# tkeskita/smoothMesh

Hardware: AMD Instinct MI355X
Metric: mesh-points smoothed/sec/node (100 iters) + achieved HBM GB/s vs roofline (higher is better)
Workload: dtype f64

## Files before the change

### smoothmesh_amd/csrc/smgpu.hip

```cpp
#include <hip/hip_runtime.h>
#include <hip/hip_ext.h>

#include <algorithm>
#include <chrono>
#include <future>
#include <memory>
#include <mutex>
#include <cstdio>
#include <cstring>
#include <string>
#include <vector>

#include "kernels.hpp"
#include "layers.hpp"
#include "kernels_tiled.hpp"
#include "kernels_walk.hpp"
#include "kernels_filter.hpp"
#include "kernels_boundary.hpp"
#include "kernels_quality.hpp"
#include "boundary.hpp"
#include "tiles.hpp"
#include "topology.hpp"
#include "parallel.hpp"

// ... 154 lines not shown
    hipStream_t bndSide = nullptr;
    hipEvent_t evBndFork = nullptr, evBndJoin = nullptr;
    bool bndPreInFlight = false;
    bool bndPending = false, bndNormalsFromLayers = false;
    std::vector<double> bndPts, bndSurfPts;
    std::vector<int32_t> bndSurfTris;
    std::vector<uint8_t> bndFlags, bndInternal;
    std::vector<BndPatch> bndPatches;
    double bndBlend = 0.0;
    BndView bv{};
    BoundarySetup bs;
    std::vector<int32_t> layerHopsHost, layerMapHost;
    bool useExch = false;
    hipStream_t exch = nullptr;
    hipEvent_t evToExch = nullptr, evFromExch = nullptr;
    bool faFilterInFlight = false;
    EdgeTiles etl;
    EdgeTileView ev{};
    bool edgeTilesOk = false;
    size_t avgPackedCount = 0;
    size_t edgeLds = 0;
    bool eaCoop = true;
    int eaMaxEntries = 0;
    int *qOwn = nullptr, *qNei = nullptr;
    QFace* qFacePart = nullptr;
    QCell* qCellPart = nullptr;
    smgpu_quality* qOut = nullptr;
    int *qProcFace = nullptr, *qSlot = nullptr;
    int qNProc = 0, qNotCounted = 0, qCountedProc = 0;
    std::vector<int32_t> qCoupling;
    smgpu_quality_part* qPartOut = nullptr;
    uint64_t qEpoch = 1, qPackEpoch = 0;
    bool iterOpen = false;
};

static int envInt(const char* name, int def) {
    const char* v = std::getenv(name);
    return v ? std::atoi(v) : def;
}

static int sideStreamDefault(int64_t nPoints) {
    const char* v = std::getenv("ROCPROF_COUNTER_COLLECTION");
    if (v && std::atoi(v) != 0) return 0;
    return nPoints <= (int64_t)envInt("SMGPU_SIDE_STREAM_MAX_POINTS", 4000000) ? 1 : 0;
}


template <typename T>
static int devAlloc(smgpu_handle* h, T** out, size_t n) {
    void* p = nullptr;
    const size_t bytes = std::max<size_t>(n, 1) * sizeof(T);
    HIP_OK(hipMalloc(&p, bytes));
    h->allocs.push_back(p);
    h->deviceBytes += (int64_t)bytes;
    *out = (T*)p;
    return 0;
}
template <typename T>
static int devUpload(smgpu_handle* h, const T** out, const std::vector<T>& v) {
    T* p = nullptr;
    if (devAlloc(h, &p, v.size())) return 1;
    if (!v.empty()) HIP_OK(hipMemcpy(p, v.data(), v.size() * sizeof(T), hipMemcpyHostToDevice));
    *out = p;
    return 0;
}

static Prm makePrm(const smgpu_handle* h) {
    const smgpu_params& p = h->prm;
    Prm r;
    r.layersOn = h->layersOn ? 1 : 0;
    r.bndOn = h->bndOn ? 1 : 0;
    r.maxStep = p.maxStepLength;
    r.relStepFrac = p.relStepFrac;
    r.minEdge = p.minEdgeLength;
    r.totalMinFreeze = p.totalMinFreeze;
    r.smallAngle = SMGPU_PI * p.minAngle / 180.0;
    r.largeAngle = SMGPU_PI * p.maxAngle / 180.0;
    const double M = (double)kFaMargin + 2.0e-5;
    r.faCosLo = (r.smallAngle >= SMGPU_PI) ? -2.0f : (float)(std::cos(std::max(r.smallAngle, 0.0)) - M);
    r.faCosHi = (r.largeAngle <= 0.0) ? 2.0f : (float)(std::cos(std::min(r.largeAngle, SMGPU_PI)) + M);
    static const long long nearUlps = [] { const char* e = std::getenv("SMGPU_NEARTIE_ULPS"); return e ? std::max(0ll, std::atoll(e)) : 4ll; }();
    r.nearUlps = nearUlps;
    return r;
}

static inline int gridFor(int64_t n) { return (int)((n + kBlock - 1) / kBlock); }

template <typename F>
static int launchK(smgpu_handle* h, int k, F&& f, hipStream_t stream = nullptr) {
    if (!stream) stream = h->stream;
    if (h->timing) {
        hipEvent_t a, b;
        for (hipEvent_t* ev : {&a, &b}) {
            if (!h->freeEvents.empty()) { *ev = h->freeEvents.back(); h->freeEvents.pop_back(); }
            else HIP_OK(hipEventCreate(ev));
        }
        HIP_OK(hipEventRecord(a, stream));
        f();
        HIP_OK(hipEventRecord(b, stream));
        h->pending.push_back({k, a, b});
    } else {
        f();
    }
    const hipError_t le = hipGetLastError();
    if (le != hipSuccess) return fail(std::string("launch of ") + kKernelNames[k] + ": " + hipGetErrorString(le));
    h->launches[k]++;
    return 0;
}

template <typename F>
static int launchKDispatch(smgpu_handle* h, int k, F&& f) {
    if (h->timing) {
        hipEvent_t a, b;
        for (hipEvent_t* ev : {&a, &b}) {
            if (!h->freeEvents.empty()) { *ev = h->freeEvents.back(); h->freeEvents.pop_back(); }
            else HIP_OK(hipEventCreate(ev));
        }
        f(a, b);
        h->pending.push_back({k, a, b});
    } else {
        f((hipEvent_t) nullptr, (hipEvent_t) nullptr);
    }
    const hipError_t le = hipGetLastError();
    if (le != hipSuccess) return fail(std::string("launch of ") + kKernelNames[k] + ": " + hipGetErrorString(le));
    h->launches[k]++;
    return 0;
}

static hipError_t zeroNow(void* p, int v, size_t bytes) {
    hipError_t e = hipMemset(p, v, bytes);
    return e != hipSuccess ? e : hipStreamSynchronize(nullptr);
}

enum { DEP_FORK = 0, DEP_JOIN = 1, DEP_TO_EXCH = 2, DEP_FROM_EXCH = 3, DEP_BND_FORK = 4, DEP_BND_JOIN = 5, DEP_COUNT = 6 };
static int depInit(smgpu_handle* h) {
    if (h->depWords || !envInt("SMGPU_STREAM_OPS", 1)) return 0;
    int can = 0;
    if (hipDeviceGetAttribute(&can, hipDeviceAttributeCanUseStreamWaitValue, h->device) != hipSuccess || !can) { (void)hipGetLastError(); return 0; }
    if (hipMalloc((void**)&h->depWords, DEP_COUNT * 64) != hipSuccess) { (void)hipGetLastError(); h->depWords = nullptr; return 0; }
    if (zeroNow(h->depWords, 0, DEP_COUNT * 64) != hipSuccess) return fail("hipMemset failed");
    h->streamOps = true;
    return 0;
}
static int depSignal(smgpu_handle* h, int kind, hipStream_t from, hipEvent_t ev) {
    if (h->streamOps) {
        if (hipStreamWriteValue32(from, h->depWords + 16 * kind, ++h->depValue[kind], 0) == hipSuccess) return 0;
        (void)hipGetLastError();
        h->streamOps = false;
    }
    HIP_OK(hipEventRecord(ev, from));
    return 0;
}
static int depWait(smgpu_handle* h, int kind, hipStream_t to, hipEvent_t ev) {
    if (h->streamOps) { HIP_OK(hipStreamWaitValue32(to, h->depWords + 16 * kind, h->depValue[kind], hipStreamWaitValueGte, 0xffffffffu)); }
    else HIP_OK(hipStreamWaitEvent(to, ev, 0));
    return 0;
}

static int drainTimers(smgpu_handle* h) {
    if (h->pending.empty()) return 0;
    HIP_OK(hipStreamSynchronize(h->stream));
    if (h->side) HIP_OK(hipStreamSynchronize(h->side));
    if (h->bndSide) HIP_OK(hipStreamSynchronize(h->bndSide));
    for (auto& p : h->pending) {
        float ms = 0.f;
        HIP_OK(hipEventElapsedTime(&ms, p.a, p.b));
        h->ms[p.k] += ms;
        h->freeEvents.push_back(p.a);
        h->freeEvents.push_back(p.b);
    }
    h->pending.clear();
    return 0;
}

static bool swapApplyOn(const smgpu_handle* h) {
    return (h->prm.edgeAngleConstraint || h->prm.faceAngleConstraint) && h->useTiles && !h->bndOn && !h->haloOn && h->dStepSqr &&
           envInt("SMGPU_APPLY_SWAP", 1);
}

static bool swapApplyHalo(const smgpu_handle* h) {
    return (h->prm.edgeAngleConstraint || h->prm.faceAngleConstraint) && h->useTiles && !h->bndOn && !h->layersOn && h->haloOn && h->dStepSqr &&
           envInt("SMGPU_APPLY_SWAP", 1);
}

static void computeAlgoBytes(smgpu_handle* h) {
    const Topology& t = h->topo;
    const int64_t P = t.nPoints, C = t.nCells, F = t.nFaces, E = t.nEdges;
    const int64_t nfp = t.facePoints.nnz(), npc = t.pointCells.nnz(), npp = (int64_t)t.pointPoints.size(), npf = t.facePoints.nnz();
    const int64_t nef = t.edgeFaces.nnz(), nec = t.edgeCells.nnz(), ncf = t.cellFacesGeom.nnz();
    const bool fa = h->prm.faceAngleConstraint;
    int64_t* b = h->algoBytes;
    b[K_FACE_GEOM] = 24 * P + 4 * (F + 1) + 4 * nfp + 48 * F + (fa ? 24 * F : 0);
    b[K_CELL_CENTRES] = 4 * (C + 1) + 4 * ncf + 48 * F + 24 * C;
    const int64_t smooth = 4 * (P + 1) + 4 * npc + 24 * C + 4 * (P + 1) + 4 * npp + 24 * P + P + 24 * P;
    b[K_SMOOTH_FINAL] = smooth;
    b[K_SMOOTH_PROP] = smooth + P + (swapApplyOn(h) ? 8 * P : 0);
    b[K_EDGE_ANGLE] = 4 * (P + 1) + 8 * npf + 24 * P + 24 * P + 2 * P;
    b[K_FA_EDGES] = 8 * E + 4 * (E + 1) + 4 * nef + 4 * (E + 1) + 6 * nec + 24 * P + 24 * F + 24 * C + 16 * E;
    b[K_FA_POINTS] = 4 * (P + 1) + 4 * npp + 16 * E + 16 * P + P;
    b[K_FA_PRED] = P;
    b[K_FA_WALK] = P;
    b[K_APPLY] = swapApplyOn(h) ? 8 * P + 2 * P : 24 * P + 24 * P + 2 * P + 24 * P;
    b[K_FINISH] = 64;
    b[K_HALO] = 0;
    b[K_BND] = 0;
    b[K_GEOM_TILE] = 24 * P + 4 * (F + 1) + 4 * nfp + 4 * (C + 1) + 4 * ncf + 24 * C + (fa ? 24 * F : 0);
    b[K_EA_FILTER] = b[K_EDGE_ANGLE];
    b[K_FA_FILTER] = b[K_FA_EDGES] - 16 * E + E + 4 * (P + 1) + 4 * npp + P;
    int64_t ops = 0;
    for (int32_t f = 0; f < t.nFaces; ++f) {
        const int64_t n = t.facePoints.off[f + 1] - t.facePoints.off[f];
        ops += (n == 3) ? 27 : 3 * (n - 1) + (((n & (n - 1)) == 0) ? 3 : 33) + 58 * n + 39;
    }
    for (int32_t c = 0; c < t.nCells; ++c) {
        const int64_t k = t.cellFacesGeom.off[c + 1] - t.cellFacesGeom.off[c];
        ops += 3 * (k - 1) + (((k & (k - 1)) == 0) ? 3 : 33) + 24 * k + 33;
    }
    for (int k = 0; k < K_COUNT; ++k) h->algoF64[k] = 0;
    h->algoF64[K_GEOM_TILE] = ops;
}

static size_t maxTileTotal(int nTiles, std::initializer_list<const std::vector<int32_t>*> offs) {
    size_t mx = 0;
    for (int t = 0; t < nTiles; ++t) {
        size_t n = 0;
        for (const std::vector<int32_t>* o : offs) n += (size_t)((*o)[(size_t)t + 1] - (*o)[(size_t)t]);
        mx = std::max(mx, n);
    }
    return mx;
}
static int defaultGeomCapWeighted(int T) { return (T == 256 && SMGPU_GEOM_WAVES >= 5) ? 3980 : 0x7fffffff; }
static int defaultSmoothCapTotal(int T) { return T == 256 ? 1112 : 0x7fffffff; }
static int defaultEdgeCapTotal() { return 852; }

static int uploadSmoothView(smgpu_handle* h, const SmoothTiles& st, SmoothTileView& v, int usePairShare) {
    int rc = 0;
    rc |= devUpload(h, &v.ptOrder, st.order);
    rc |= devUpload(h, &v.ptBeg, st.ptBeg);
    rc |= devUpload(h, &v.tcOff, st.tcOff);
    rc |= devUpload(h, &v.tcIds, st.tcIds);
    rc |= devUpload(h, &v.tnOff, st.tnOff);
    rc |= devUpload(h, &v.tnIds, st.tnIds);
    rc |= devUpload(h, &v.selfLoc, st.selfLoc);
    rc |= devUpload(h, &v.pcBase, st.pcBase);
    rc |= devUpload(h, &v.pcWidth, st.pcWidth);
    rc |= devUpload(h, &v.pcEll, st.pcEll);
    rc |= devUpload(h, &v.ppBase, st.ppBase);
    rc |= devUpload(h, &v.ppWidth, st.ppWidth);
    rc |= devUpload(h, &v.ppEll, st.ppEll);
    rc |= devUpload(h, &v.pairEll, st.pairEll);
    rc |= devUpload(h, &v.pfBase, st.pfBase);
    rc |= devUpload(h, &v.pfWidth, st.pfWidth);
    rc |= devUpload(h, &v.pfEll, st.pfEll);
    std::vector<int> meta((size_t)kSmoothMetaInts * (size_t)std::max(st.nTiles, 1), 0);
    for (int t = 0; t < st.nTiles; ++t) {
        int* r = meta.data() + (size_t)kSmoothMetaInts * t;
        r[0] = st.ptBeg[t]; r[1] = st.ptBeg[t + 1] - st.ptBeg[t]; r[2] = st.tcOff[t]; r[3] = st.tcOff[t + 1] - st.tcOff[t];
        r[4] = st.tnOff[t]; r[5] = st.tnOff[t + 1] - st.tnOff[t]; r[6] = st.pcBase[t]; r[7] = st.pcWidth[t];
        r[8] = st.ppBase[t]; r[9] = st.ppWidth[t]; r[10] = st.pfBase[t]; r[11] = st.pfWidth[t];
    }
    rc |= devUpload(h, &v.meta, meta);
    v.maxCells = st.maxCells; v.maxPoints = st.maxPoints;
    v.usePairShare = usePairShare;
    return rc;
}

extern "C" {

const char* smgpu_last_error(void) { return g_err.c_str(); }
const char* smgpu_version(void) { return "smgpu 0.1 (gfx950)"; }

static int ensureHostLists(smgpu_handle* h, int groups) {
    if (!h->devLists.valid) return 0;
    std::string why;
    return downloadDeferredLists(h->topo, h->devLists, h->device, why, groups) ? fail("device -> host copy of the addressing: " + why) : 0;
}

static void freeOwnerNeighbour(DeviceTopologyArrays& dt) {
    for (DeviceTopologyArrays::Arr* a : {&dt.owner, &dt.neighbour})
        if (a->p) { (void)hipFree(a->p); a->p = nullptr; a->bytes = 0; }
}
static void freeDevTopo(DeviceTopologyArrays& dt) {
    freeOwnerNeighbour(dt);
    for (DeviceTopologyArrays::Arr* a : {&dt.faceOff, &dt.facePts, &dt.cfOff, &dt.cfVal, &dt.pcOff, &dt.pcVal, &dt.ppOff, &dt.ppPt, &dt.peEdge, &dt.pfOff, &dt.pfFace,
                                         &dt.pfPrev, &dt.pfNext, &dt.pfPrevSlot, &dt.pfNextSlot, &dt.ringFace, &dt.ringCell, &dt.edgeRingOk, &dt.edges, &dt.efOff,
                                         &dt.efFace, &dt.ecOff, &dt.ecCell, &dt.ecF0, &dt.ecF1})
        if (a->p) { (void)hipFree(a->p); a->p = nullptr; a->bytes = 0; }
    dt.valid = false;
}

int smgpu_create(const smgpu_mesh_desc* d, smgpu_handle** out) {
    if (!d || !out) return fail("smgpu_create: null argument");
    *out = nullptr;
    int nDev = 0;
    if (hipGetDeviceCount(&nDev) != hipSuccess || nDev <= 0) return fail("smgpu_create: no HIP device available");
    if (d->device < 0 || d->device >= nDev) return fail("smgpu_create: device ordinal out of range");
    smgpu_handle* h = new smgpu_handle();
    h->device = d->device;
    const auto tCreate0 = std::chrono::steady_clock::now();
    setupClockStart() = tCreate0;
    auto sinceCreate = [&] { return std::chrono::duration<double>(std::chrono::steady_clock::now() - tCreate0).count(); };
    const bool wantTiles = envInt("SMGPU_TILES", 1) != 0;
    const bool mortonTiles = envInt("SMGPU_TILE_MORTON", 1) != 0;
    std::future<std::vector<int32_t>> fPointOrder;
    if (wantTiles && mortonTiles) fPointOrder = std::async(std::launch::async, [&] { return mortonOrderOf(d->nPoints, d->points); });
    std::future<std::string> fGeom, fSmooth, fEdge;
    std::function<void()> startEdge;
    CornerChains chains;
    struct ChainsGuard { CornerChains& c; std::future<std::string>& f; ~ChainsGuard() { if (f.valid()) f.wait(); releaseCornerChains(c); } } chainsGuard{chains, fSmooth};
    static const char* const kHostTablesPending = "\x01host tables pending";
    std::vector<int32_t> pointOrder;
    std::vector<uint8_t> internalMask;
    DeviceTopologyArrays devTopo;
    {
        const int geomT0 = envInt("SMGPU_GEOM_T", 256), smoothT0 = envInt("SMGPU_SMOOTH_T", 256);
        const int geomCells0 = envInt("SMGPU_GEOM_CELLS", geomT0 / 2);
        const int capGP0 = envInt("SMGPU_GEOM_CAPP", std::min(6 * geomCells0, 1400)), capGF0 = envInt("SMGPU_GEOM_CAPF", std::min(4 * geomCells0, 1400));
        const int capSC0 = envInt("SMGPU_SMOOTH_CAPC", std::min(2 * smoothT0, 1500)), capSN0 = envInt("SMGPU_SMOOTH_CAPN", std::min(3 * smoothT0, 1500));
        const bool geomOk = geomT0 == 64 || geomT0 == 128 || geomT0 == 256, smoothOk = smoothT0 == 64 || smoothT0 == 128 || smoothT0 == 256;
        const bool devTiles = envInt("SMGPU_DEVICE_TILES", 1) != 0;
        const auto afterCells = [&] {
                      if (wantTiles && geomOk && smoothOk && devTiles && devTopo.valid && envInt("SMGPU_DEVICE_TILES", 1) == 1) {
                          std::string why;
                          if (startCornerChains(devTopo, d->nPoints, h->device, chains, why) == 2) chains = CornerChains();
                      }
                      if (wantTiles && geomOk) fGeom = std::async(std::launch::async, [&, geomT0, geomCells0, capGP0, capGF0, devTiles]() -> std::string {
                      std::vector<int32_t> cellOrder;
                      if (mortonTiles && devTiles && devTopo.valid && envInt("SMGPU_DEVICE_TILES", 1) == 1) {
                          std::string why;
                          if (cellMortonOrderOnDevice(devTopo, d->nCells, d->nPoints, d->points, h->device, cellOrder, why) != 0) cellOrder.clear();
                      }
                      const std::string e = h->gt.buildBoundaries(h->topo, d->points, mortonTiles, geomT0, geomCells0, capGP0, capGF0,
                                                                  envInt("SMGPU_GEOM_CAPWEIGHTED", defaultGeomCapWeighted(geomT0)), SMGPU_GEOM_AOS ? kGF : 6,
                                                                  cellOrder.empty() ? nullptr : &cellOrder);
                      if (!e.empty()) return e;
                      if (devTopo.valid && !devTiles) return std::string(kHostTablesPending);
                      if (devTopo.valid) {
                          std::string why;
                          const auto t0 = std::chrono::steady_clock::now();
                          const int rc = envInt("SMGPU_DEVICE_TILES", 1) == 2 ? 1 : buildGeomTablesOnDevice(h->gt, devTopo, d->nCells, h->device, h->gtDev, why);
                          if (envInt("SMGPU_VERBOSE", 0) >= 2)
                              std::fprintf(stderr, "[smgpu] geometry tiles: tables on the %s %.2f s   (done at +%.3f s)\n", rc == 0 ? "device" : "host (device build handed them back)",
                                           std::chrono::duration<double>(std::chrono::steady_clock::now() - t0).count(), setupClock());
                          if (rc == 0) return std::string();
                          return rc == 2 ? "device tile tables: " + why : std::string(kHostTablesPending);
                      }
                      return h->gt.buildTables(h->topo); }); };
        const auto afterPoints = [&] {
                if (!(wantTiles && geomOk && smoothOk)) return;
                if (fPointOrder.valid()) pointOrder = fPointOrder.get();
                internalMask.resize((size_t)d->nPoints);
                for (int p = 0; p < d->nPoints; ++p) internalMask[(size_t)p] = d->isInternalPoint[p] ? 1 : 0;
                h->isInternalHost = internalMask;
                fSmooth = std::async(std::launch::async, [&, smoothT0, capSC0, capSN0, devTiles]() -> std::string {
                    const std::string e = h->stl.buildBoundaries(h->topo, d->points, mortonTiles, smoothT0, capSC0, capSN0, (mortonTiles && !pointOrder.empty()) ? &pointOrder : nullptr, nullptr,
                                                                  envInt("SMGPU_SMOOTH_CAPTOTAL", defaultSmoothCapTotal(smoothT0)));
                    if (!e.empty()) return e;
                    if (devTopo.valid && !devTiles) return std::string(kHostTablesPending);
                    if (devTopo.valid) {
                        std::string why;
                        const auto t0 = std::chrono::steady_clock::now();
                        const int rc = envInt("SMGPU_DEVICE_TILES", 1) == 2 ? 1 : buildSmoothTablesOnDevice(h->stl, devTopo, d->nPoints, h->topo.maxPointPoints, internalMask.data(), h->device, h->stDev, why, &chains);
                        if (envInt("SMGPU_VERBOSE", 0) >= 2)
                            std::fprintf(stderr, "[smgpu] smoothing tiles: tables on the %s %.2f s   (done at +%.3f s)\n", rc == 0 ? "device" : "host (device build handed them back)",
                                         std::chrono::duration<double>(std::chrono::steady_clock::now() - t0).count(), setupClock());
                        if (rc == 0) return std::string();
                        return rc == 2 ? "device tile tables: " + why : std::string(kHostTablesPending);
                    }
                    return h->stl.buildTables(h->topo, internalMask.data()); });
            };
        startEdge = [&, devTiles] {
            if (!wantTiles) return;
            if (fPointOrder.valid()) pointOrder = fPointOrder.get();
            const std::vector<int32_t>* po = (mortonTiles && !pointOrder.empty()) ? &pointOrder : nullptr;
            const bool wantFilter = envInt("SMGPU_FILTER", 1) != 0;
            const bool devTilesE = devTiles && devTopo.valid, devLists = devTopo.valid;
            const DeviceTopologyArrays* dt = &devTopo;
            fEdge = std::async(std::launch::async, [h, d, po, wantFilter, mortonTiles, devTilesE, devLists, dt]() -> std::string {
                if (!wantFilter) return std::string("not built");
                const std::string e = h->etl.buildBoundaries(h->topo, d->points, mortonTiles, 256, envInt("SMGPU_EDGE_CAPP", 512), envInt("SMGPU_EDGE_CAPF", 768), envInt("SMGPU_EDGE_CAPC", 512), po,
                                                                  envInt("SMGPU_EDGE_CAPTOTAL", defaultEdgeCapTotal()));
                if (!e.empty()) return e;
                if (devLists && !devTilesE) return std::string(kHostTablesPending);
                if (devTilesE) {
                    std::string why;
                    const auto t0 = std::chrono::steady_clock::now();
                    const int rc = envInt("SMGPU_DEVICE_TILES", 1) == 2 ? 1 : buildEdgeTablesOnDevice(h->etl, *dt, h->topo.nEdges, h->device, h->etDev, why);
                    if (envInt("SMGPU_VERBOSE", 0) >= 2)
                        std::fprintf(stderr, "[smgpu] edge tiles: tables on the %s %.2f s   (done at +%.3f s)\n", rc == 0 ? "device" : "host (device build handed them back)",
                                     std::chrono::duration<double>(std::chrono::steady_clock::now() - t0).count(), setupClock());
                    if (rc == 0) return std::string();
                    return rc == 2 ? "device tile tables: " + why : std::string(kHostTablesPending);
                }
                return h->etl.buildTables(h->topo);
            });
        };
        std::string terr;
        int dev = envInt("SMGPU_DEVICE_TOPOLOGY", 1) ? 1 : -1;
        if (dev > 0) {
            std::string why;
            dev = buildTopologyOnDevice(h->topo, d->nPoints, d->nCells, d->nFaces, d->nInternalFaces, d->faceOffsets, d->facePoints, d->owner, d->neighbour, h->device, why,
                                        afterCells, afterPoints, &devTopo, startEdge, devTiles && wantTiles);
            if (dev == 2) {
                if (fGeom.valid()) fGeom.wait();
                if (fSmooth.valid()) fSmooth.wait();
                if (fEdge.valid()) fEdge.wait();
                if (fPointOrder.valid()) fPointOrder.wait();
                freeDevTopo(devTopo);
                delete h;
                return fail("smgpu_create: device addressing: " + why);
            }
            if (envInt("SMGPU_VERBOSE", 0) >= 1) std::fprintf(stderr, "[smgpu] addressing on the %s (%.2f s since create)\n", dev == 0 ? "device" : "host (device path handed the mesh back)", sinceCreate());
        }
        if (dev != 0) {
            h->topo = Topology();
            terr = h->topo.build(d->nPoints, d->nCells, d->nFaces, d->nInternalFaces, d->faceOffsets, d->facePoints, d->owner, d->neighbour, afterCells, afterPoints);
        }
        if (!terr.empty()) {
            if (fGeom.valid()) fGeom.wait();
            if (fSmooth.valid()) fSmooth.wait();
            if (fPointOrder.valid()) fPointOrder.wait();
            delete h;
            return fail("smgpu_create: " + terr);
        }
        if (!fEdge.valid()) startEdge();
    }
    bool devAdopted = false;
    auto cleanup = [&](int rc) {
        if (fGeom.valid()) fGeom.wait();
        if (fSmooth.valid()) fSmooth.wait();
        if (fPointOrder.valid()) fPointOrder.wait();
        if (fEdge.valid()) fEdge.wait();
        if (!devAdopted) freeDevTopo(devTopo);
        else freeOwnerNeighbour(devTopo);
        smgpu_destroy(h);
        return rc;
    };
    if (hipSetDevice(h->device) != hipSuccess) return cleanup(fail("hipSetDevice failed"));
    if (d->useCallerStream) h->stream = (hipStream_t)d->stream;
    else {
        if (hipStreamCreateWithFlags(&h->stream, hipStreamNonBlocking) != hipSuccess) return cleanup(fail("hipStreamCreate failed"));
        h->ownStream = true;
    }
    const Topology& t = h->topo;
    MeshView& m = h->mv;
    const double tTopo = sinceCreate();
    double tLap = tTopo;
    auto lapC = [&](const char* what) { if (envInt("SMGPU_VERBOSE", 0) >= 2) { const double now = sinceCreate(); std::fprintf(stderr, "[smgpu] create: %-28s %.3f s   (at +%.3f s)\n", what, now - tLap, now); tLap = now; } };
    auto cleanupE = [&](int rc0) { if (fEdge.valid()) fEdge.wait(); return cleanup(rc0); };
    m.nPoints = t.nPoints; m.nCells = t.nCells; m.nFaces = t.nFaces; m.nInternalFaces = t.nInternalFaces; m.nEdges = t.nEdges;
    std::vector<uint8_t> flags(t.nPoints);
    for (int p = 0; p < t.nPoints; ++p)
        flags[p] = (d->isInternalPoint[p] ? PF_INTERNAL : 0) |
                   ((d->isSmoothingSurfacePoint && d->isSmoothingSurfacePoint[p]) ? PF_SMOOTHSURF : 0);
    int rc = 0;
    auto adopt = [&](auto*& dst, const DeviceTopologyArrays::Arr& a) { dst = (std::remove_reference_t<decltype(dst)>)a.p; h->allocs.push_back(a.p); h->deviceBytes += (int64_t)a.bytes; };
    if (devTopo.valid) {
        devAdopted = true;
        h->devLists = devTopo;
        adopt(m.faceOff, devTopo.faceOff);
        adopt(m.facePts, devTopo.facePts);
        adopt(m.cfOff, devTopo.cfOff);
        adopt(m.cfVal, devTopo.cfVal);
        adopt(m.pcOff, devTopo.pcOff);
        adopt(m.pcVal, devTopo.pcVal);
        adopt(m.ppOff, devTopo.ppOff);
        adopt(m.ppPt, devTopo.ppPt);
        adopt(m.peEdge, devTopo.peEdge);
        adopt(m.pfOff, devTopo.pfOff);
        adopt(m.pfFace, devTopo.pfFace);
        adopt(m.pfPrev, devTopo.pfPrev);
        adopt(m.pfNext, devTopo.pfNext);
        adopt(m.pfPrevSlot, devTopo.pfPrevSlot);
        adopt(m.pfNextSlot, devTopo.pfNextSlot);
        adopt(m.ringFace, devTopo.ringFace);
        adopt(m.ringCell, devTopo.ringCell);
        adopt(m.edgeRingOk, devTopo.edgeRingOk);
        adopt(m.edges, devTopo.edges);
        adopt(m.efOff, devTopo.efOff);
        adopt(m.efFace, devTopo.efFace);
        adopt(m.ecOff, devTopo.ecOff);
        adopt(m.ecCell, devTopo.ecCell);
        adopt(m.ecF0, devTopo.ecF0);
        adopt(m.ecF1, devTopo.ecF1);
    } else {
        rc |= devUpload(h, &m.faceOff, t.facePoints.off);
        rc |= devUpload(h, &m.facePts, t.facePoints.val);
        rc |= devUpload(h, &m.cfOff, t.cellFacesGeom.off);
        rc |= devUpload(h, &m.cfVal, t.cellFacesGeom.val);
        rc |= devUpload(h, &m.pcOff, t.pointCells.off);
        rc |= devUpload(h, &m.pcVal, t.pointCells.val);
        rc |= devUpload(h, &m.ppOff, t.pointEdges.off);
        rc |= devUpload(h, &m.ppPt, t.pointPoints);
        rc |= devUpload(h, &m.peEdge, t.pointEdges.val);
        rc |= devUpload(h, &m.pfOff, t.pointFaces.off);
        rc |= devUpload(h, &m.pfFace, t.pointFaces.val);
        rc |= devUpload(h, &m.pfPrev, t.pfPrev);
        rc |= devUpload(h, &m.pfNext, t.pfNext);
        rc |= devUpload(h, &m.pfPrevSlot, t.pfPrevSlot);
        rc |= devUpload(h, &m.pfNextSlot, t.pfNextSlot);
        rc |= devUpload(h, &m.ringFace, t.ringFace);
        rc |= devUpload(h, &m.ringCell, t.ringCell);
        rc |= devUpload(h, &m.edgeRingOk, t.edgeRingOk);
        rc |= devUpload(h, &m.edges, t.edges);
        rc |= devUpload(h, &m.efOff, t.edgeFaces.off);
        rc |= devUpload(h, &m.efFace, t.edgeFaces.val);
        rc |= devUpload(h, &m.ecOff, t.edgeCells.off);
        rc |= devUpload(h, &m.ecCell, t.edgeCells.val);
        rc |= devUpload(h, &m.ecF0, t.ecFace0);
        rc |= devUpload(h, &m.ecF1, t.ecFace1);
    }
    rc |= devUpload(h, &m.pflags, flags);
    if (rc) return cleanupE(1);
    lapC("addressing adopted / uploaded");
    h->useTiles = envInt("SMGPU_TILES", 1) != 0;
    h->useFilter = envInt("SMGPU_FILTER", 1) != 0;
    h->xcdMap = envInt("SMGPU_XCD_MAP", 1) != 0;
    h->walkStar = envInt("SMGPU_WALK_STAR", 1) != 0;
    h->starBlocks = std::max(1, envInt("SMGPU_STAR_BLOCKS", 256 * 32));
    h->walkPack = envInt("SMGPU_WALK_PACK", 1) != 0;
    h->walkCache = envInt("SMGPU_WALK_CACHE", 1) != 0;
    h->faLists = envInt("SMGPU_FA_LISTS", 1) != 0;
    h->faSideExact = envInt("SMGPU_FA_SIDE_EXACT", 1) != 0;
    h->bndInGeom = envInt("SMGPU_BND_IN_GEOM", 1) != 0;
    { const char* fv = std::getenv("SMGPU_FOAM_VARIANT"); h->foamOrg = fv && std::string(fv) == "org"; }
    { const char* sv = std::getenv("SMGPU_SYNC_VARIANT"); h->st.ownFold = (sv && std::string(sv) == "own") ? 1 : 0; }
    if (h->useTiles) {
        h->geomT = envInt("SMGPU_GEOM_T", 256);
        h->smoothT = envInt("SMGPU_SMOOTH_T", 256);
        if (h->geomT != 64 && h->geomT != 128 && h->geomT != 256) return cleanupE(fail("SMGPU_GEOM_T must be 64, 128 or 256"));
        if (h->smoothT != 64 && h->smoothT != 128 && h->smoothT != 256) return cleanupE(fail("SMGPU_SMOOTH_T must be 64, 128 or 256"));
        const int geomCells = envInt("SMGPU_GEOM_CELLS", h->geomT / 2);
        const int capGP = envInt("SMGPU_GEOM_CAPP", std::min(6 * geomCells, 1400));
        const int capGF = envInt("SMGPU_GEOM_CAPF", std::min(4 * geomCells, 1400));
        const int capSC = envInt("SMGPU_SMOOTH_CAPC", std::min(2 * h->smoothT, 1500));
        const int capSN = envInt("SMGPU_SMOOTH_CAPN", std::min(3 * h->smoothT, 1500));
        (void)geomCells; (void)capGP; (void)capGF; (void)capSC; (void)capSN;
        std::string e2 = fSmooth.valid() ? fSmooth.get() : std::string("not built");
        std::string e1 = fGeom.valid() ? fGeom.get() : std::string("not built");
        std::string e3 = fEdge.valid() ? fEdge.get() : std::string("not built");
        if (e1 == kHostTablesPending) e1 = h->gt.buildTables(h->topo);
        std::string whyD;
        if (e2 == kHostTablesPending) e2 = downloadDeferredLists(h->topo, devTopo, h->device, whyD, 1) ? "device -> host copy of the addressing: " + whyD : h->stl.buildTables(h->topo, internalMask.data());
        if (e3 == kHostTablesPending) e3 = downloadDeferredLists(h->topo, devTopo, h->device, whyD, 2) ? "device -> host copy of the addressing: " + whyD : h->etl.buildTables(h->topo);
        if (envInt("SMGPU_VERBOSE", 0))
            std::fprintf(stderr, "[smgpu] set-up: addressing %.2f s, tile tables (3 host threads) %.2f s\n", tTopo, sinceCreate() - tTopo);
        freeOwnerNeighbour(devTopo);
        lapC("tile tasks joined");
        if (!e1.empty() || !e2.empty()) {
            h->useTiles = false;
        } else {
            GeomTileView& g = h->gv;
            SmoothTileView& v = h->sv;
            auto adoptT = [&](auto*& dst, const GeomTilesDev::Arr& a) { dst = (std::remove_reference_t<decltype(dst)>)a.p; h->allocs.push_back(a.p); h->deviceBytes += (int64_t)a.bytes; };
            if (h->gtDev.valid) {
                adoptT(g.cellOrder, h->gtDev.cellOrder); adoptT(g.cellBeg, h->gtDev.cellBeg); adoptT(g.tpIds, h->gtDev.tpIds); adoptT(g.tfIds, h->gtDev.tfIds);
                adoptT(g.faceVerts, h->gtDev.faceVerts); adoptT(g.cellFaces, h->gtDev.cellFaces); adoptT(g.meta, h->gtDev.meta);
                h->gtDev.valid = false;
            } else {
                rc |= devUpload(h, &g.cellOrder, h->gt.order);
                rc |= devUpload(h, &g.cellBeg, h->gt.cellBeg);
                rc |= devUpload(h, &g.tpIds, h->gt.tpIds);
                rc |= devUpload(h, &g.tfIds, h->gt.tfIds);
                rc |= devUpload(h, &g.faceVerts, h->gt.faceVerts);
                rc |= devUpload(h, &g.cellFaces, h->gt.cellFaces);
            }
            rc |= devUpload(h, &g.tpOff, h->gt.tpOff);
            rc |= devUpload(h, &g.tfOff, h->gt.tfOff);
            rc |= devUpload(h, &g.fvBase, h->gt.fvBase);
            rc |= devUpload(h, &g.fvWidth, h->gt.fvWidth);
            rc |= devUpload(h, &g.cfBase, h->gt.cfBase);
            rc |= devUpload(h, &g.cfWidth, h->gt.cfWidth);
            rc |= devUpload(h, &g.tileFlags, h->gt.tileFlags);
            if (!g.meta) {
                const auto& gt = h->gt;
                std::vector<int> meta((size_t)kGeomMetaInts * (size_t)gt.nTiles, 0);
                for (int t = 0; t < gt.nTiles; ++t) {
                    int* r = meta.data() + (size_t)kGeomMetaInts * t;
                    r[0] = gt.tpOff[t]; r[1] = gt.tpOff[t + 1] - gt.tpOff[t]; r[2] = gt.tfOff[t]; r[3] = gt.tfOff[t + 1] - gt.tfOff[t];
                    r[4] = gt.fvBase[t]; r[5] = gt.fvWidth[t]; r[6] = gt.cellBeg[t]; r[7] = gt.cellBeg[t + 1] - gt.cellBeg[t];
                    r[8] = gt.cfBase[t]; r[9] = gt.cfWidth[t]; r[10] = gt.tileFlags[t];
                }
                rc |= devUpload(h, &g.meta, meta);
            }
            g.maxPoints = h->gt.maxPoints; g.maxFaces = h->gt.maxFaces;
            if (h->stDev.valid) {
                auto adoptS = [&](auto*& dst, const SmoothTilesDev::Arr& a) { dst = (std::remove_reference_t<decltype(dst)>)a.p; h->allocs.push_back(a.p); h->deviceBytes += (int64_t)a.bytes; };
                adoptS(v.ptOrder, h->stDev.order); adoptS(v.ptBeg, h->stDev.ptBeg); adoptS(v.tcIds, h->stDev.tcIds); adoptS(v.tnIds, h->stDev.tnIds); adoptS(v.selfLoc, h->stDev.selfLoc);
                adoptS(v.pcEll, h->stDev.pcEll); adoptS(v.ppEll, h->stDev.ppEll); adoptS(v.pairEll, h->stDev.pairEll); adoptS(v.pfEll, h->stDev.pfEll); adoptS(v.meta, h->stDev.meta);
                h->stDev.valid = false;
            } else {
                rc |= devUpload(h, &v.ptOrder, h->stl.order);
                rc |= devUpload(h, &v.ptBeg, h->stl.ptBeg);
                rc |= devUpload(h, &v.tcIds, h->stl.tcIds);
                rc |= devUpload(h, &v.tnIds, h->stl.tnIds);
                rc |= devUpload(h, &v.selfLoc, h->stl.selfLoc);
                rc |= devUpload(h, &v.pcEll, h->stl.pcEll);
                rc |= devUpload(h, &v.ppEll, h->stl.ppEll);
                rc |= devUpload(h, &v.pairEll, h->stl.pairEll);
                rc |= devUpload(h, &v.pfEll, h->stl.pfEll);
            }
            rc |= devUpload(h, &v.tcOff, h->stl.tcOff);
            rc |= devUpload(h, &v.tnOff, h->stl.tnOff);
            rc |= devUpload(h, &v.pcBase, h->stl.pcBase);
            rc |= devUpload(h, &v.pcWidth, h->stl.pcWidth);
            rc |= devUpload(h, &v.ppBase, h->stl.ppBase);
            rc |= devUpload(h, &v.ppWidth, h->stl.ppWidth);
            rc |= devUpload(h, &v.pfBase, h->stl.pfBase);
            rc |= devUpload(h, &v.pfWidth, h->stl.pfWidth);
            if (!v.meta) {
                const auto& st = h->stl;
                std::vector<int> meta((size_t)kSmoothMetaInts * (size_t)st.nTiles, 0);
                for (int t = 0; t < st.nTiles; ++t) {
                    int* r = meta.data() + (size_t)kSmoothMetaInts * t;
                    r[0] = st.ptBeg[t]; r[1] = st.ptBeg[t + 1] - st.ptBeg[t]; r[2] = st.tcOff[t]; r[3] = st.tcOff[t + 1] - st.tcOff[t];
                    r[4] = st.tnOff[t]; r[5] = st.tnOff[t + 1] - st.tnOff[t]; r[6] = st.pcBase[t]; r[7] = st.pcWidth[t];
                    r[8] = st.ppBase[t]; r[9] = st.ppWidth[t]; r[10] = st.pfBase[t]; r[11] = st.pfWidth[t];
                }
                rc |= devUpload(h, &v.meta, meta);
            }
            v.maxCells = h->stl.maxCells; v.maxPoints = h->stl.maxPoints;
            v.usePairShare = t.maxPointPoints <= 16 ? 1 : 0;
            if (h->useFilter) {
                if (e3.empty()) {
                    EdgeTileView& ev = h->ev;
                    const size_t nGeomTf = (size_t)h->gt.tfOff.back();
                    h->avgPackedCount = nGeomTf;
                    if (h->etDev.valid) {
                        std::string why;
                        if (remapEdgeFaceIdsOnDevice(g.tfIds, (long long)nGeomTf, t.nFaces, (int*)h->etDev.tfIds.p, h->etDev.nTf, h->device, why))
                            return cleanup(fail("smgpu_create: edge tile face positions: " + why));
                        auto adoptE = [&](auto*& dst, const EdgeTilesDev::Arr& a) { dst = (std::remove_reference_t<decltype(dst)>)a.p; h->allocs.push_back(a.p); h->deviceBytes += (int64_t)a.bytes; };
                        adoptE(ev.order, h->etDev.order); adoptE(ev.edgeBeg, h->etDev.edgeBeg); adoptE(ev.tpIds, h->etDev.tpIds); adoptE(ev.tfIds, h->etDev.tfIds);
                        adoptE(ev.tcIds, h->etDev.tcIds); adoptE(ev.epLoc, h->etDev.epLoc); adoptE(ev.efEll, h->etDev.efEll); adoptE(ev.ecEll, h->etDev.ecEll);
                        adoptE(ev.meta, h->etDev.meta);
                        h->etDev.valid = false;
                    } else {
                        if (h->gt.tfIds.size() != nGeomTf) {
                            h->gt.tfIds.resize(nGeomTf);
                            if (hipMemcpy(h->gt.tfIds.data(), g.tfIds, nGeomTf * 4, hipMemcpyDeviceToHost) != hipSuccess) return cleanup(fail("smgpu_create: download of the tile face ids failed"));
                        }
                        std::vector<int32_t> facePos((size_t)t.nFaces, -1);
                        for (size_t k = 0; k < h->gt.tfIds.size(); ++k)
                            if (h->gt.tfIds[k] < 0) facePos[(size_t)(h->gt.tfIds[k] & 0x7fffffff)] = (int32_t)k;
                        for (int32_t& f : h->etl.tfIds) f = facePos[(size_t)f];
                        rc |= devUpload(h, &ev.order, h->etl.order);
                        rc |= devUpload(h, &ev.edgeBeg, h->etl.edgeBeg);
                        rc |= devUpload(h, &ev.tpIds, h->etl.tpIds);
                        rc |= devUpload(h, &ev.tfIds, h->etl.tfIds);
                        rc |= devUpload(h, &ev.tcIds, h->etl.tcIds);
                        rc |= devUpload(h, &ev.epLoc, h->etl.epLoc);
                        rc |= devUpload(h, &ev.efEll, h->etl.efEll);
                        rc |= devUpload(h, &ev.ecEll, h->etl.ecEll);
                    }
                    rc |= devUpload(h, &ev.tpOff, h->etl.tpOff);
                    rc |= devUpload(h, &ev.tfOff, h->etl.tfOff);
                    rc |= devUpload(h, &ev.tcOff, h->etl.tcOff);
                    rc |= devUpload(h, &ev.efBase, h->etl.efBase);
                    rc |= devUpload(h, &ev.ecBase, h->etl.ecBase);
                    rc |= devUpload(h, &ev.efWidth, h->etl.efWidth);
                    rc |= devUpload(h, &ev.ecWidth, h->etl.ecWidth);
                    if (!ev.meta) {
                        const auto& et = h->etl;
                        std::vector<int> meta((size_t)kEdgeMetaInts * (size_t)et.nTiles, 0);
                        for (int ti = 0; ti < et.nTiles; ++ti) {
                            int* r = meta.data() + (size_t)kEdgeMetaInts * ti;
                            r[0] = et.edgeBeg[ti]; r[1] = et.edgeBeg[ti + 1] - et.edgeBeg[ti]; r[2] = et.tpOff[ti]; r[3] = et.tpOff[ti + 1] - et.tpOff[ti];
                            r[4] = et.tfOff[ti]; r[5] = et.tfOff[ti + 1] - et.tfOff[ti]; r[6] = et.tcOff[ti]; r[7] = et.tcOff[ti + 1] - et.tcOff[ti];
                            r[8] = et.efBase[ti]; r[9] = et.efWidth[ti]; r[10] = et.ecBase[ti]; r[11] = et.ecWidth[ti];
                        }
                        rc |= devUpload(h, &ev.meta, meta);
                    }
                    ev.maxPoints = h->etl.maxPoints; ev.maxFaces = h->etl.maxFaces; ev.maxCells = h->etl.maxCells;
                    h->edgeLds = sizeof(double) * 3 * maxTileTotal(h->etl.nTiles, {&h->etl.tpOff, &h->etl.tfOff, &h->etl.tcOff});
                    h->edgeTilesOk = h->edgeLds <= 64 * 1024;
                    if (envInt("SMGPU_VERBOSE", 0))
                        std::fprintf(stderr, "[smgpu] edge tiles: n=%d LDS=%zu B (maxP %d maxF %d maxC %d)\n", h->etl.nTiles, h->edgeLds, ev.maxPoints, ev.maxFaces, ev.maxCells);
                    if (h->edgeTilesOk && envInt("SMGPU_SIDE_STREAM", sideStreamDefault(t.nPoints))) {
                        if (depInit(h)) return cleanup(1);
                        if (hipStreamCreateWithFlags(&h->side, hipStreamNonBlocking) != hipSuccess ||
                            hipEventCreateWithFlags(&h->evFork, hipEventDisableTiming) != hipSuccess ||
                            hipEventCreateWithFlags(&h->evJoin, hipEventDisableTiming) != hipSuccess)
                            return cleanup(fail("side stream creation failed"));
                    }
                }
            }
            if (rc) return cleanup(1);
            {
                size_t mx = 0;
                for (int ti = 0; ti < h->gt.nTiles; ++ti)
                    mx = std::max(mx, 3 * (size_t)(h->gt.tpOff[(size_t)ti + 1] - h->gt.tpOff[(size_t)ti]) +
                                          (size_t)(SMGPU_GEOM_AOS ? kGF : 6) * (size_t)(h->gt.tfOff[(size_t)ti + 1] - h->gt.tfOff[(size_t)ti]));
                h->geomLds = sizeof(double) * mx;
            }
            h->smoothLds = sizeof(double) * 3 * maxTileTotal(h->stl.nTiles, {&h->stl.tcOff, &h->stl.tnOff});
            if (envInt("SMGPU_VERBOSE", 0))
                std::fprintf(stderr, "[smgpu] tiles: geom T=%d n=%d LDS=%zu B (maxP %d maxF %d; staged faces x%.3f, points x%.3f of the mesh's)  smooth T=%d n=%d LDS=%zu B (maxC %d maxN %d)\n",
                             h->geomT, h->gt.nTiles, h->geomLds, g.maxPoints, g.maxFaces, (double)h->gt.tfOff.back() / std::max(1, t.nFaces),
                             (double)h->gt.tpOff.back() / std::max(1, t.nPoints), h->smoothT, h->stl.nTiles, h->smoothLds, v.maxCells, v.maxPoints);
        }
    }
    {
        const char* ea = std::getenv("SMGPU_EDGE_ANGLE");
        h->eaCoop = !(ea && std::string(ea) == "faithful");
        for (int p0 = 0; p0 < t.nPoints; p0 += kEaPointsPerBlock) {
            const int p1 = std::min(t.nPoints, p0 + kEaPointsPerBlock);
            h->eaMaxEntries = std::max(h->eaMaxEntries, t.pointEdges.off[p1] - t.pointEdges.off[p0]);
        }
        if (sizeof(double) * 9 * (size_t)h->eaMaxEntries > 60 * 1024) h->eaCoop = false;
    }
    lapC("tile tables adopted / uploaded");
    State& s = h->st;
    const size_t P = t.nPoints, C = t.nCells, F = t.nFaces, E = t.nEdges;
    rc |= devAlloc(h, &h->bufA, 3 * P);
    rc |= devAlloc(h, &h->bufB, 3 * P);
    rc |= devAlloc(h, &s.prop, 3 * P);
    rc |= devAlloc(h, &h->dStepSqr, P + 4);
    rc |= devAlloc(h, &s.fCtr, 3 * F);
    rc |= devAlloc(h, &s.fArea, 3 * F);
    s.avgPacked = (h->useTiles && h->edgeTilesOk && h->avgPackedCount) ? 1 : 0;
    rc |= devAlloc(h, &s.fAvg, 3 * (s.avgPacked ? h->avgPackedCount : F));
    rc |= devAlloc(h, &s.cellCtr, 3 * C);
    rc |= devAlloc(h, &s.frozen, P);
    rc |= devAlloc(h, &s.edgeMin, E);
    rc |= devAlloc(h, &s.edgeMax, E);
    rc |= devAlloc(h, &s.ptMin, P);
    rc |= devAlloc(h, &s.ptMax, P);
    rc |= devAlloc(h, &s.faActive, P + 16);
    rc |= devAlloc(h, &h->dFaMaybe, P + 16);
    rc |= devAlloc(h, &s.faEdgeList, E);
    rc |= devAlloc(h, &s.faPointList, P);
    rc |= devAlloc(h, &h->dEaMaybe, P);
    rc |= devAlloc(h, &s.faS, P);
    rc |= devAlloc(h, &s.faN, t.pointPoints.size());
    rc |= devAlloc(h, &s.walkStack, P + 64);
    rc |= devAlloc(h, &s.acc, 1);
    rc |= devAlloc(h, &s.nearTotal, 4);
    {
        const size_t nPart = (size_t)std::max(gridFor(t.nPoints), h->useTiles ? h->stl.nTiles : 0) + 2 * (size_t)gridFor(t.nPoints) + 1;
        rc |= devAlloc(h, &s.blkMax, nPart);
        rc |= devAlloc(h, &s.blkCnt, nPart);
    }
    if (rc) return cleanup(1);
    lapC("work arrays allocated");
    if (hipMemset(s.acc, 0, sizeof(Accum)) != hipSuccess) return cleanup(fail("hipMemset failed"));
    if (hipMemsetAsync(s.nearTotal, 0, 4 * sizeof(unsigned long long), h->stream) != hipSuccess) return cleanup(fail("hipMemset failed"));
    if (hipMemset(s.frozen, 0, P) != hipSuccess) return cleanup(fail("hipMemset failed"));
    if (hipMemcpy(h->bufA, d->points, 3 * P * sizeof(double), hipMemcpyHostToDevice) != hipSuccess)
        return cleanup(fail("upload of points failed"));
    if (hipMemcpy(s.prop, h->bufA, 3 * P * sizeof(double), hipMemcpyDeviceToDevice) != hipSuccess)
        return cleanup(fail("upload of points failed"));
    lapC("points uploaded");
    s.ptsCur = h->bufA;
    s.ptsNext = h->bufB;
    s.stats = nullptr;
    s.sharedSlot = nullptr;
    s.combA = nullptr;
    {
        void* dp = nullptr;
        if (hipHostMalloc((void**)&h->nActiveHost, 64, hipHostMallocMapped) == hipSuccess &&
            hipHostGetDevicePointer(&dp, h->nActiveHost, 0) == hipSuccess) {
            *(volatile int*)h->nActiveHost = -1;
            s.nActiveHost = (int*)dp;
        } else {
            (void)hipGetLastError();
            if (h->nActiveHost) (void)hipHostFree(h->nActiveHost);
            h->nActiveHost = nullptr;
            s.nActiveHost = nullptr;
        }
    }
    computeAlgoBytes(h);
    if (fEdge.valid()) fEdge.wait();
    freeOwnerNeighbour(devTopo);
    h->devLists.owner = h->devLists.neighbour = DeviceTopologyArrays::Arr();
    if (envInt("SMGPU_VERBOSE", 0)) std::fprintf(stderr, "[smgpu] set-up: total %.2f s\n", sinceCreate());
    *out = h;
    return 0;
}

int smgpu_destroy(smgpu_handle* h) {
    if (!h) return 0;
    (void)hipSetDevice(h->device);
    if (h->stream) (void)hipStreamSynchronize(h->stream);
    for (auto& p : h->pending) { (void)hipEventDestroy(p.a); (void)hipEventDestroy(p.b); }
    for (auto e : h->freeEvents) (void)hipEventDestroy(e);
    for (void* p : h->allocs) (void)hipFree(p);
    if (h->stDev.valid)
        for (const SmoothTilesDev::Arr* a : {&h->stDev.order, &h->stDev.ptBeg, &h->stDev.tcIds, &h->stDev.tnIds, &h->stDev.selfLoc, &h->stDev.pcEll, &h->stDev.ppEll, &h->stDev.pairEll, &h->stDev.pfEll, &h->stDev.meta})
            if (a->p) (void)hipFree(a->p);
    if (h->etDev.valid)
        for (const EdgeTilesDev::Arr* a : {&h->etDev.order, &h->etDev.edgeBeg, &h->etDev.tpIds, &h->etDev.tfIds, &h->etDev.tcIds, &h->etDev.epLoc, &h->etDev.efEll, &h->etDev.ecEll, &h->etDev.meta})
            if (a->p) (void)hipFree(a->p);
    if (h->gtDev.valid)
        for (const GeomTilesDev::Arr* a : {&h->gtDev.cellOrder, &h->gtDev.cellBeg, &h->gtDev.tpIds, &h->gtDev.tfIds, &h->gtDev.faceVerts, &h->gtDev.cellFaces, &h->gtDev.meta})
            if (a->p) (void)hipFree(a->p);
    for (void* p : {(void*)h->qOwn, (void*)h->qNei, (void*)h->qFacePart, (void*)h->qCellPart, (void*)h->qOut, (void*)h->qProcFace, (void*)h->qSlot,
                    (void*)h->qPartOut})
        if (p) (void)hipFree(p);
    if (h->pinned) (void)hipHostFree(h->pinned);
    if (h->nActiveHost) (void)hipHostFree(h->nActiveHost);
    for (hipEvent_t e : h->evWalkLag) if (e) (void)hipEventDestroy(e);
    if (h->side) { (void)hipStreamSynchronize(h->side); (void)hipStreamDestroy(h->side); }
    if (h->evToExch) (void)hipEventDestroy(h->evToExch);
    if (h->evFromExch) (void)hipEventDestroy(h->evFromExch);
    if (h->depWords) (void)hipFree(h->depWords);
    if (h->bndSide) { (void)hipStreamSynchronize(h->bndSide); (void)hipStreamDestroy(h->bndSide); }
    if (h->evBndFork) (void)hipEventDestroy(h->evBndFork);
    if (h->evBndJoin) (void)hipEventDestroy(h->evBndJoin);
    if (h->evFork) (void)hipEventDestroy(h->evFork);
    if (h->evJoin) (void)hipEventDestroy(h->evJoin);
    if (h->ownStream && h->stream) (void)hipStreamDestroy(h->stream);
    delete h;
    return 0;
}

int smgpu_get_sizes(smgpu_handle* h, smgpu_sizes* o) {
    if (!h || !o) return fail("null argument");
    const Topology& t = h->topo;
    o->nPoints = t.nPoints; o->nCells = t.nCells; o->nFaces = t.nFaces; o->nInternalFaces = t.nInternalFaces; o->nEdges = t.nEdges;
    o->nnzFacePoints = t.facePoints.nnz(); o->nnzPointCells = t.pointCells.nnz(); o->nnzPointPoints = (int64_t)t.pointPoints.size();
    o->nnzPointFaces = t.facePoints.nnz(); o->nnzEdgeFaces = t.edgeFaces.nnz(); o->nnzEdgeCells = t.edgeCells.nnz();
    o->nnzCellFaces = t.cellFacesGeom.nnz();
    o->deviceBytes = h->deviceBytes;
    return 0;
}

int smgpu_mesh_stats(smgpu_handle* h, double* minEdge, double* maxEdge) {
    if (!h) return fail("null handle");
    HIP_OK(hipSetDevice(h->device));
    unsigned long long* d = nullptr;
    HIP_OK(hipMalloc((void**)&d, 16));
    struct Release { void* p; ~Release() { if (p) (void)hipFree(p); } } release{d};
    const double big = 1.0e300, zero = 0.0;
    unsigned long long init[2];
    std::memcpy(&init[0], &big, 8);
    std::memcpy(&init[1], &zero, 8);
    HIP_OK(hipMemcpyAsync(d, init, 16, hipMemcpyHostToDevice, h->stream));
    hipLaunchKernelGGL(k_edge_stats, dim3(std::max(1, std::min(gridFor(h->mv.nEdges), 1024))), dim3(kBlock), 0, h->stream, h->mv, h->st.ptsCur, d, d + 1);
    unsigned long long out[2];
    HIP_OK(hipMemcpyAsync(out, d, 16, hipMemcpyDeviceToHost, h->stream));
    HIP_OK(hipStreamSynchronize(h->stream));
    std::memcpy(minEdge, &out[0], 8);
    std::memcpy(maxEdge, &out[1], 8);
    return 0;
}

namespace smgpu {
__device__ __forceinline__ uint64_t mix64(uint64_t z) {
    z += 0x9E3779B97F4A7C15ull; z = (z ^ (z >> 30)) * 0xBF58476D1CE4E5B9ull; z = (z ^ (z >> 27)) * 0x94D049BB133111EBull;
    return z ^ (z >> 31);
}
__device__ __forceinline__ double selftestArg(uint64_t seed, long i, int j) {
    const uint64_t r = mix64(seed + 8ull * (uint64_t)i + (uint64_t)j);
    const uint64_t mant = r & 0xFFFFFFFFFFFFFull, sign = r >> 63;
    const unsigned pick = (unsigned)((r >> 52) & 0x7ff);
    uint64_t expo;
    switch ((i + (j == 3 ? 0 : 0)) & 7) {
        case 0: case 1: case 2: expo = 1023 - 40 + pick % 80; break;
        case 3: return __longlong_as_double((long long)r);
        case 4: {
            const unsigned k = pick % 6;
            if (k == 0) return sign ? -0.0 : 0.0;
            if (k == 1) return __longlong_as_double((long long)((sign << 63) | mant));
            if (k == 2) return __longlong_as_double((long long)((sign << 63) | (0x7ffull << 52)));
            if (k == 3) return __longlong_as_double((long long)((0x7ffull << 52) | mant | 1));
            expo = 1 + pick % 60; break;
        }
        case 5: {
            const unsigned edges[6] = {1023 - 767, 1023 - 250, 1023 + 250, 2046, 1, 1023 - 969};
            expo = edges[pick % 6] + (pick / 6) % 5 - 2;
            if ((long long)expo < 1) expo = 1;
            if (expo > 2046) expo = 2046;
            break;
        }
        case 6: expo = 1 + pick % 2046; break;
        default: expo = 1023 - 300 + pick % 600; break;
    }
    const uint64_t sgn = (j == 0 && (i & 8)) ? 0 : sign;
    return __longlong_as_double((long long)((sgn << 63) | (expo << 52) | mant));
}
__device__ __forceinline__ bool sameBits(double a, double b) { return (a != a && b != b) || __double_as_longlong(a) == __double_as_longlong(b); }
__global__ void k_selftest_fpexact(uint64_t seed, long n, unsigned long long* bad) {
    unsigned long long mine = 0;
    for (long i = blockIdx.x * (long)blockDim.x + threadIdx.x; i < n; i += (long)gridDim.x * blockDim.x) {
        const double x = selftestArg(seed, i, 0), y = selftestArg(seed, i, 1), z = selftestArg(seed, i, 2), w = selftestArg(seed, i, 3);
        if (!sameBits(sqrtExact(x), sqrt(x))) ++mine;
        double a0, a1, a2, a3;
        sqrtExact4(fabs(x), fabs(y), z, fabs(w), a0, a1, a2, a3);
        if (!sameBits(a0, sqrt(fabs(x))) || !sameBits(a1, sqrt(fabs(y))) || !sameBits(a2, sqrt(z)) || !sameBits(a3, sqrt(fabs(w)))) ++mine;
        const V3 q = divExact(v3(x, y, z), w);
        if (!sameBits(q.x, x / w) || !sameBits(q.y, y / w) || !sameBits(q.z, z / w)) ++mine;
        const V3 q6 = divExact(v3(x, y, z), 6.0);
        if (!sameBits(q6.x, x / 6.0) || !sameBits(q6.y, y / 6.0) || !sameBits(q6.z, z / 6.0)) ++mine;
    }
    if (mine) atomicAdd(bad, mine);
}
}

int smgpu_debug_selftest_fpexact(int32_t device, uint64_t seed, int64_t n, int64_t* mismatches) {
    if (!mismatches || n < 0) return fail("smgpu_debug_selftest_fpexact: bad arguments");
    if (hipSetDevice(device) != hipSuccess) return fail("smgpu_debug_selftest_fpexact: hipSetDevice failed");
    unsigned long long* d = nullptr;
    if (hipMalloc(&d, sizeof(*d)) != hipSuccess) return fail("smgpu_debug_selftest_fpexact: hipMalloc failed");
    unsigned long long host = 0;
    bool ok = hipMemset(d, 0, sizeof(*d)) == hipSuccess;
    if (ok) {
        hipLaunchKernelGGL(smgpu::k_selftest_fpexact, dim3(2048), dim3(256), 0, 0, seed, (long)n, d);
        ok = hipGetLastError() == hipSuccess && hipMemcpy(&host, d, sizeof(host), hipMemcpyDeviceToHost) == hipSuccess;
    }
    (void)hipFree(d);
    if (!ok) return fail("smgpu_debug_selftest_fpexact: launch failed");
    *mismatches = (int64_t)host;
    return 0;
}

int smgpu_set_foam_variant(smgpu_handle* h, int32_t variant) {
    if (!h) return fail("null handle");
    if (variant != SMGPU_FOAM_COM && variant != SMGPU_FOAM_ORG) return fail("smgpu_set_foam_variant: unknown variant");
    h->foamOrg = variant == SMGPU_FOAM_ORG;
    h->qEpoch++;
    h->geomAheadDone = false;
    return 0;
}

int smgpu_set_sync_variant(smgpu_handle* h, int32_t variant) {
    if (!h) return fail("null handle");
    if (variant != SMGPU_SYNC_MASTER && variant != SMGPU_SYNC_OWN) return fail("smgpu_set_sync_variant: unknown variant");
    h->st.ownFold = variant == SMGPU_SYNC_OWN ? 1 : 0;
    return 0;
}

int smgpu_set_params(smgpu_handle* h, const smgpu_params* p) {
    if (!h || !p) return fail("null argument");
    if (!(p->maxStepLength > 0.0)) return fail("maxStepLength must be > 0");
    h->prm = *p;
    h->prmSet = true;
    h->walkMode = -1;
    h->walkSwitches = 0;
    h->walkDecisions = 0;
    if (h->nActiveHost) *(volatile int*)h->nActiveHost = -1;
    h->geomAheadDone = false;
    computeAlgoBytes(h);
    return 0;
}

extern "C++" {
template <typename K>
static void ensureDynLds(K kernel, int device, size_t bytes) {
    static std::mutex mu;
    static size_t have[64] = {0};
    if (bytes <= 64 * 1024 || device < 0 || device >= 64) return;
    std::lock_guard<std::mutex> lock(mu);
    if (have[device] >= bytes) return;
    if (hipFuncSetAttribute((const void*)kernel, hipFuncAttributeMaxDynamicSharedMemorySize, (int)bytes) == hipSuccess) have[device] = bytes;
    else (void)hipGetLastError();
}
template <int T, bool ORG>
static void launchGeomTileAs(smgpu_handle* h, const MeshView& m, const State& s, int wantAvg, const int* tileList, int nTiles, hipEvent_t evA, hipEvent_t evB,
                             bool withBndPre) {
    if (withBndPre) {
        const int nNormal = (h->bv.nB + T - 1) / T, nFeat = (h->bv.nFeat + (T / 64) - 1) / (T / 64);
        const int nBnd = ((nNormal + nFeat + 7) / 8) * 8;
        ensureDynLds(k_geom_tile_bnd<T, ORG>, h->device, h->geomLds);
        hipExtLaunchKernelGGL((k_geom_tile_bnd<T, ORG>), dim3(nBnd + tileGrid(nTiles, h->xcdMap)), dim3(T), (uint32_t)h->geomLds, h->stream, evA, evB, 0, m, s, h->gv,
                              wantAvg, h->writeFaces ? 1 : 0, tileList, nTiles, h->xcdMap, h->deferN, h->deferIter, h->deferLocal, h->deferHist, h->bv, nBnd, nNormal);
    } else {
        ensureDynLds(k_geom_tile<T, ORG>, h->device, h->geomLds);
        hipExtLaunchKernelGGL((k_geom_tile<T, ORG>), dim3(tileGrid(nTiles, h->xcdMap)), dim3(T), (uint32_t)h->geomLds, h->stream, evA, evB, 0, m, s, h->gv, wantAvg,
                              h->writeFaces ? 1 : 0, tileList, nTiles, h->xcdMap, h->deferN, h->deferIter, h->deferLocal, h->deferHist);
    }
    h->deferN = 0;
    h->deferLocal = h->deferHist = nullptr;
}
template <int T>
static void launchGeomTile(smgpu_handle* h, const MeshView& m, const State& s, int wantAvg, const int* tileList, int nTiles, hipEvent_t evA, hipEvent_t evB,
// ... 2294 lines not shown
```

### smoothmesh_amd/csrc/tiles.cpp

```cpp
#include "tiles.hpp"
#include "parallel.hpp"

#include <algorithm>
#include <chrono>
#include <cstdio>
#include <cstdlib>

namespace smgpu {

namespace {
struct PhaseTimer {
    const char* who;
    bool on;
    std::chrono::steady_clock::time_point t;
    explicit PhaseTimer(const char* w) : who(w), on(std::getenv("SMGPU_VERBOSE") && std::atoi(std::getenv("SMGPU_VERBOSE")) >= 2), t(std::chrono::steady_clock::now()) {}
    void lap(const char* what) {
        const auto now = std::chrono::steady_clock::now();
        if (on) std::fprintf(stderr, "[smgpu] %s tiles: %-18s %.2f s   (done at +%.3f s)\n", who, what, std::chrono::duration<double>(now - t).count(), setupClock());
        t = now;
    }
};
}


static inline int32_t roundUp4(int32_t v) { return v <= 4 ? 4 : (v + 3) & ~3; }

static inline uint64_t spread21(uint64_t v) {
    v &= 0x1fffff;
    v = (v | v << 32) & 0x1f00000000ffffull;
    v = (v | v << 16) & 0x1f0000ff0000ffull;
    v = (v | v << 8) & 0x100f00f00f00f00full;
    v = (v | v << 4) & 0x10c30c30c30c30c3ull;
    v = (v | v << 2) & 0x1249249249249249ull;
    return v;
}

static std::vector<int32_t> mortonOrder(int32_t n, const double* xyz) {
    double lo[3] = {1e300, 1e300, 1e300}, hi[3] = {-1e300, -1e300, -1e300};
    {
        const int parts = rangeParts(n);
        std::vector<double> plo(3 * (size_t)parts, 1e300), phi(3 * (size_t)parts, -1e300);
        parallelRanges(n, parts, [&](int part, int64_t b, int64_t e) {
            double l[3] = {1e300, 1e300, 1e300}, h[3] = {-1e300, -1e300, -1e300};
            for (int64_t i = b; i < e; ++i)
                for (int a = 0; a < 3; ++a) { l[a] = std::min(l[a], xyz[3 * (size_t)i + a]); h[a] = std::max(h[a], xyz[3 * (size_t)i + a]); }
            for (int a = 0; a < 3; ++a) { plo[3 * (size_t)part + a] = l[a]; phi[3 * (size_t)part + a] = h[a]; }
        });
        for (int part = 0; part < parts; ++part)
            for (int a = 0; a < 3; ++a) { lo[a] = std::min(lo[a], plo[3 * (size_t)part + a]); hi[a] = std::max(hi[a], phi[3 * (size_t)part + a]); }
    }
    double ext = 0.0;
    for (int a = 0; a < 3; ++a) ext = std::max(ext, hi[a] - lo[a]);
    const double scale = ext > 0.0 ? 2097151.0 / ext : 0.0;
    std::vector<std::pair<uint64_t, int32_t>> key((size_t)n);
    parallelRanges(n, rangeParts(n), [&](int, int64_t b, int64_t e) {
        for (int64_t i = b; i < e; ++i) {
            uint64_t k = 0;
            for (int a = 0; a < 3; ++a) k |= spread21((uint64_t)((xyz[3 * (size_t)i + a] - lo[a]) * scale)) << a;
            key[(size_t)i] = {k, (int32_t)i};
        }
    });
    if (rangeParts(n) > 1) {
        const int shift = 55;
        std::vector<size_t> cnt(257, 0);
        for (int32_t i = 0; i < n; ++i) ++cnt[(size_t)(key[(size_t)i].first >> shift) + 1];
        for (int bkt = 0; bkt < 256; ++bkt) cnt[(size_t)bkt + 1] += cnt[(size_t)bkt];
        std::vector<std::pair<uint64_t, int32_t>> tmp((size_t)n);
        {
            std::vector<size_t> cur(cnt.begin(), cnt.end() - 1);
            for (int32_t i = 0; i < n; ++i) tmp[cur[(size_t)(key[(size_t)i].first >> shift)]++] = key[(size_t)i];
        }
        key.swap(tmp);
        std::vector<std::pair<uint64_t, int32_t>>().swap(tmp);
        parallelRanges(256, (int)std::min<unsigned>(hostThreads(), 256u), [&](int, int64_t b, int64_t e) {
            for (int64_t bkt = b; bkt < e; ++bkt) std::sort(key.begin() + (ptrdiff_t)cnt[(size_t)bkt], key.begin() + (ptrdiff_t)cnt[(size_t)bkt + 1]);
        });
    } else std::sort(key.begin(), key.end());
    std::vector<int32_t> order((size_t)n);
    for (int32_t i = 0; i < n; ++i) order[(size_t)i] = key[(size_t)i].second;
    return order;
}

std::vector<int32_t> mortonOrderOf(int32_t n, const double* xyz) { return mortonOrder(n, xyz); }

static std::vector<int32_t> naturalOrder(int32_t n) {
    std::vector<int32_t> o((size_t)n);
    for (int32_t i = 0; i < n; ++i) o[(size_t)i] = i;
    return o;
}

std::string GeomTiles::build(const Topology& t, const double* pts, bool morton, int32_t nThreads, int32_t capCells,
                             int32_t capPoints, int32_t capFaces, int32_t capWeighted, int32_t faceWeight) {
    const std::string e = buildBoundaries(t, pts, morton, nThreads, capCells, capPoints, capFaces, capWeighted, faceWeight);
    return e.empty() ? buildTables(t) : e;
}

static unsigned tileSegments() {
    static const unsigned n = [] { const char* e = std::getenv("SMGPU_TILE_SEGMENTS"); return e ? std::max(1u, std::min((unsigned)std::atoi(e), 64u)) : 16u; }();
    return n;
}
struct Stamps {
    int32_t* p;
    size_t bytes;
    explicit Stamps(size_t n) : bytes(std::max<size_t>(n, 1) * sizeof(int32_t)) {
        void* m = ::mmap(nullptr, bytes, PROT_READ | PROT_WRITE, MAP_PRIVATE | MAP_ANONYMOUS, -1, 0);
        if (m == MAP_FAILED) throw std::bad_alloc();
        p = (int32_t*)m;
        adviseHuge(m, bytes);
    }
    ~Stamps() { ::munmap(p, bytes); }
    Stamps(const Stamps&) = delete;
    Stamps& operator=(const Stamps&) = delete;
    int32_t& operator[](size_t i) { return p[i]; }
};

std::string GeomTiles::buildBoundaries(const Topology& t, const double* pts, bool morton, int32_t nThreads, int32_t capCells,
                                       int32_t capPoints, int32_t capFaces, int32_t capWeighted, int32_t faceWeight, const std::vector<int32_t>* cellOrder) {
    threads = nThreads;
    PhaseTimer tm("geometry");
    if (capCells > threads) capCells = threads;
    const auto& cf = t.cellFacesGeom;
    const auto& fp = t.facePoints;
    if (morton && cellOrder && (int64_t)cellOrder->size() == t.nCells) order = *cellOrder;
    else if (morton) {
        std::vector<double> cc(3 * (size_t)t.nCells, 0.0);
        parallelRanges(t.nCells, rangeParts(t.nCells), [&](int, int64_t cb0, int64_t ce0) {
            for (int32_t c = (int32_t)cb0; c < (int32_t)ce0; ++c) {
                double s[3] = {0, 0, 0};
                int32_t n = 0;
                for (int32_t k = cf.off[c]; k < cf.off[c + 1]; ++k) {
                    const int32_t f = cf.val[k] & 0x7fffffff;
                    for (int32_t j = fp.off[f]; j < fp.off[f + 1]; ++j, ++n)
                        for (int a = 0; a < 3; ++a) s[a] += pts[3 * (size_t)fp.val[j] + a];
                }
                for (int a = 0; a < 3; ++a) cc[3 * (size_t)c + a] = n ? s[a] / n : 0.0;
            }
        });
        order = mortonOrder(t.nCells, cc.data());
    } else order = naturalOrder(t.nCells);
    tm.lap("order");
    {
        const int segs = (t.nCells >= (2 << 20)) ? (int)std::min<unsigned>(hostThreads(), tileSegments()) : 1;
        std::vector<std::vector<int32_t>> segBeg((size_t)segs);
        std::vector<std::string> segErr((size_t)segs);
        parallelRanges(t.nCells, segs, [&](int sg, int64_t c0, int64_t c1) {
            Stamps stampP((size_t)t.nPoints), stampF((size_t)t.nFaces);
            std::vector<int32_t>& beg = segBeg[(size_t)sg];
            int32_t tile = 1, nP = 0, nF = 0, nC = 0;
            for (int32_t ci = (int32_t)c0; ci < (int32_t)c1; ++ci) {
                const int32_t c = order[(size_t)ci];
                for (int attempt = 0; attempt < 2; ++attempt) {
                    int32_t addF = 0, addP = 0;
                    for (int32_t k = cf.off[c]; k < cf.off[c + 1]; ++k) {
                        const int32_t f = cf.val[k] & 0x7fffffff;
                        if (stampF[f] != tile) { stampF[f] = tile; ++addF; }
                        for (int32_t j = fp.off[f]; j < fp.off[f + 1]; ++j)
                            if (stampP[fp.val[j]] != tile) { stampP[fp.val[j]] = tile; ++addP; }
                    }
                    if (nC > 0 && (nC + 1 > capCells || nP + addP > capPoints || nF + addF > capFaces ||
                                   3 * (int64_t)(nP + addP) + (int64_t)faceWeight * (nF + addF) > capWeighted)) {
                        beg.push_back(ci);
                        ++tile; nP = nF = nC = 0;
                        continue;
                    }
                    if (addP > capPoints || addF > capFaces) { segErr[(size_t)sg] = "a single cell exceeds the LDS tile capacity"; return; }
                    nP += addP; nF += addF; ++nC;
                    break;
                }
            }
        });
        cellBeg.assign(1, 0);
        for (int sg = 0; sg < segs; ++sg) {
            if (!segErr[(size_t)sg].empty()) return segErr[(size_t)sg];
            if (sg > 0) cellBeg.push_back((int32_t)((int64_t)t.nCells * sg / segs));
            cellBeg.insert(cellBeg.end(), segBeg[(size_t)sg].begin(), segBeg[(size_t)sg].end());
        }
        cellBeg.push_back(t.nCells);
        nTiles = (int32_t)cellBeg.size() - 1;
    }
    tm.lap("boundaries");
    return "";
}

std::string GeomTiles::buildTables(const Topology& t) {
    PhaseTimer tm("geometry");
    const auto& cf = t.cellFacesGeom;
    const auto& fp = t.facePoints;
    std::vector<int32_t> cellTile((size_t)t.nCells, -1);
    for (int32_t ti = 0; ti < nTiles; ++ti)
        for (int32_t ci = cellBeg[ti]; ci < cellBeg[ti + 1]; ++ci) cellTile[(size_t)order[(size_t)ci]] = ti;
    struct Part {
        std::vector<int32_t> tpIds, tfIds, nPts, nFcs, fvBase, cfBase;
        std::vector<uint8_t> fvWidth, cfWidth, tileFlags;
        std::vector<uint16_t> faceVerts, cellFaces;
        int32_t maxPoints = 0, maxFaces = 0;
        std::string err;
    };
    const int parts = rangeParts(nTiles, 64);
    std::vector<Part> P((size_t)parts);
    const int32_t threadsL = threads;
    parallelRanges(nTiles, parts, [&](int part, int64_t tb, int64_t te) {
        Part& o = P[(size_t)part];
        std::vector<int32_t> faces, points;
        for (int32_t ti = (int32_t)tb; ti < (int32_t)te; ++ti) {
            faces.clear(); points.clear();
            const int32_t cb = cellBeg[ti], ce = cellBeg[ti + 1];
            int32_t cw = 0, fw = 0;
            bool allQuads = true, allHex = true;
            for (int32_t ci = cb; ci < ce; ++ci) {
                const int32_t c = order[(size_t)ci];
                cw = std::max(cw, cf.off[c + 1] - cf.off[c]);
                allHex = allHex && (cf.off[c + 1] - cf.off[c] == 6);
                for (int32_t k = cf.off[c]; k < cf.off[c + 1]; ++k) faces.push_back(cf.val[k] & 0x7fffffff);
            }
            std::sort(faces.begin(), faces.end());
            faces.erase(std::unique(faces.begin(), faces.end()), faces.end());
            for (int32_t f : faces) {
                allQuads = allQuads && (fp.off[f + 1] - fp.off[f] == 4);
                fw = std::max(fw, fp.off[f + 1] - fp.off[f]);
                for (int32_t j = fp.off[f]; j < fp.off[f + 1]; ++j) points.push_back(fp.val[j]);
            }
            std::sort(points.begin(), points.end());
            points.erase(std::unique(points.begin(), points.end()), points.end());
            cw = roundUp4(cw); fw = roundUp4(fw);
            if ((int32_t)points.size() > 32767 || (int32_t)faces.size() > 32767 || cw > 252 || fw > 252) {
                o.err = "tile too large for the 15-bit local index tables";
                return;
            }
            auto locP = [&](int32_t p) { return (int32_t)(std::lower_bound(points.begin(), points.end(), p) - points.begin()); };
            auto locF = [&](int32_t f) { return (int32_t)(std::lower_bound(faces.begin(), faces.end(), f) - faces.begin()); };
            o.tpIds.insert(o.tpIds.end(), points.begin(), points.end());
            o.nPts.push_back((int32_t)points.size());
            o.fvBase.push_back((int32_t)o.faceVerts.size());
            o.fvWidth.push_back((uint8_t)fw);
            for (int32_t f : faces) {
                const bool ownerHere = cellTile[(size_t)t.owner[f]] == ti;
                o.tfIds.push_back(ownerHere ? (int32_t)(0x80000000u | (uint32_t)f) : f);
                const int32_t n = fp.off[f + 1] - fp.off[f];
                for (int32_t j = 0; j < fw; ++j) o.faceVerts.push_back(j < n ? (uint16_t)locP(fp.val[fp.off[f] + j]) : kEllPad);
            }
            o.nFcs.push_back((int32_t)faces.size());
            o.cfBase.push_back((int32_t)o.cellFaces.size());
            o.cfWidth.push_back((uint8_t)cw);
            o.tileFlags.push_back((uint8_t)((allQuads ? 1 : 0) | (allHex ? 2 : 0)));
            const size_t base = o.cellFaces.size();
            o.cellFaces.resize(base + (size_t)cw * threadsL, kEllPad);
            for (int32_t ci = cb; ci < ce; ++ci) {
                const int32_t c = order[(size_t)ci];
                const int32_t tl = ci - cb;
                for (int32_t k = cf.off[c], j = 0; k < cf.off[c + 1]; ++k, ++j) {
                    const int32_t v = cf.val[k];
                    o.cellFaces[base + ((size_t)(j / 4) * threadsL + tl) * 4 + (j % 4)] = (uint16_t)(locF(v & 0x7fffffff) | (v < 0 ? 0x8000 : 0));
                }
            }
            o.maxPoints = std::max(o.maxPoints, (int32_t)points.size());
            o.maxFaces = std::max(o.maxFaces, (int32_t)faces.size());
        }
    });
    tpOff.assign(1, 0); tfOff.assign(1, 0);
    fvBase.clear(); fvWidth.clear(); cfBase.clear(); cfWidth.clear(); tileFlags.clear();
    size_t fvTotal = 0, cfTotal = 0;
    for (Part& o : P) {
        if (!o.err.empty()) return o.err;
        for (int32_t n : o.nPts) tpOff.push_back(tpOff.back() + n);
        for (int32_t n : o.nFcs) tfOff.push_back(tfOff.back() + n);
        for (int32_t b : o.fvBase) fvBase.push_back((int32_t)(fvTotal + (size_t)b));
        for (int32_t b : o.cfBase) cfBase.push_back((int32_t)(cfTotal + (size_t)b));
        fvWidth.insert(fvWidth.end(), o.fvWidth.begin(), o.fvWidth.end());
        cfWidth.insert(cfWidth.end(), o.cfWidth.begin(), o.cfWidth.end());
        tileFlags.insert(tileFlags.end(), o.tileFlags.begin(), o.tileFlags.end());
        fvTotal += o.faceVerts.size(); cfTotal += o.cellFaces.size();
        maxPoints = std::max(maxPoints, o.maxPoints);
        maxFaces = std::max(maxFaces, o.maxFaces);
    }
    if (fvTotal > 0x7fffffffu || cfTotal > 0x7fffffffu) return "tile tables exceed int32 addressing";
    {
        std::vector<std::vector<int32_t>> a, b;
        std::vector<std::vector<uint16_t>> c, d;
        for (Part& o : P) { a.push_back(std::move(o.tpIds)); b.push_back(std::move(o.tfIds)); c.push_back(std::move(o.faceVerts)); d.push_back(std::move(o.cellFaces)); }
        concatParts(tpIds, a); concatParts(tfIds, b); concatParts(faceVerts, c); concatParts(cellFaces, d);
    }
    tm.lap("tables");
    return "";
}

namespace {
struct ChainScratch {
    std::vector<int32_t> verts, deg, adjOff, adjEdge, ea, eb, stackV, stackE, next;
    std::vector<uint8_t> used;
    std::vector<std::pair<int32_t, int32_t>> comp, out;
};
void chainCorners(std::vector<std::pair<int32_t, int32_t>>& corners, ChainScratch& w) {
    const int n = (int)corners.size();
    if (n < 2) return;
    w.verts.clear();
    for (const auto& c : corners) { w.verts.push_back(c.first); w.verts.push_back(c.second); }
    std::sort(w.verts.begin(), w.verts.end());
    w.verts.erase(std::unique(w.verts.begin(), w.verts.end()), w.verts.end());
    const int nv = (int)w.verts.size();
    auto vid = [&](int32_t v) { return (int)(std::lower_bound(w.verts.begin(), w.verts.end(), v) - w.verts.begin()); };
    w.ea.clear(); w.eb.clear();
    for (const auto& c : corners) { w.ea.push_back(vid(c.first)); w.eb.push_back(vid(c.second)); }
    w.deg.assign((size_t)nv, 0);
    for (int e = 0; e < n; ++e) { ++w.deg[(size_t)w.ea[(size_t)e]]; ++w.deg[(size_t)w.eb[(size_t)e]]; }
    int pending = -1;
    for (int v = 0; v < nv; ++v)
        if (w.deg[(size_t)v] & 1) {
            if (pending < 0) pending = v;
            else { w.ea.push_back(pending); w.eb.push_back(v); ++w.deg[(size_t)pending]; ++w.deg[(size_t)v]; pending = -1; }
        }
    const int ne = (int)w.ea.size();
    w.adjOff.assign((size_t)nv + 1, 0);
    for (int e = 0; e < ne; ++e) { ++w.adjOff[(size_t)w.ea[(size_t)e] + 1]; ++w.adjOff[(size_t)w.eb[(size_t)e] + 1]; }
    for (int v = 0; v < nv; ++v) w.adjOff[(size_t)v + 1] += w.adjOff[(size_t)v];
    w.adjEdge.assign((size_t)w.adjOff[(size_t)nv], 0);
    w.next.assign(w.adjOff.begin(), w.adjOff.end() - 1);
    for (int e = 0; e < ne; ++e) { w.adjEdge[(size_t)w.next[(size_t)w.ea[(size_t)e]]++] = e; w.adjEdge[(size_t)w.next[(size_t)w.eb[(size_t)e]]++] = e; }
    w.used.assign((size_t)ne, 0);
    std::vector<int32_t>& next = w.next;
    next.assign(w.adjOff.begin(), w.adjOff.end() - 1);
    std::vector<std::pair<int32_t, int32_t>>& out = w.out;
    out.clear();
    for (int start = 0; start < nv; ++start) {
        if (next[(size_t)start] >= w.adjOff[(size_t)start + 1]) continue;
        w.stackV.assign(1, start); w.stackE.assign(1, -1);
        std::vector<std::pair<int32_t, int32_t>>& comp = w.comp;
        comp.clear();
        while (!w.stackV.empty()) {
            const int v = w.stackV.back();
            int e = -1;
            while (next[(size_t)v] < w.adjOff[(size_t)v + 1]) {
                const int cand = w.adjEdge[(size_t)next[(size_t)v]++];
                if (!w.used[(size_t)cand]) { e = cand; break; }
            }
            if (e >= 0) {
                w.used[(size_t)e] = 1;
                const int to = (w.ea[(size_t)e] == v) ? w.eb[(size_t)e] : w.ea[(size_t)e];
                w.stackV.push_back(to); w.stackE.push_back(e);
            } else {
                const int eIn = w.stackE.back();
                w.stackV.pop_back(); w.stackE.pop_back();
                if (eIn >= 0) comp.push_back({eIn, w.stackV.back()});
            }
        }
        for (size_t i = comp.size(); i-- > 0;) {
            const int e = comp[i].first, from = comp[i].second;
            if (e >= n) continue;
            const int to = (w.ea[(size_t)e] == from) ? w.eb[(size_t)e] : w.ea[(size_t)e];
            out.push_back({w.verts[(size_t)from], w.verts[(size_t)to]});
        }
    }
    if ((int)out.size() == n) corners.swap(out);
}
}

std::string SmoothTiles::build(const Topology& t, const double* xyz, const uint8_t* isInternal, bool morton, int32_t nThreads,
                               int32_t capCells, int32_t capPoints, const std::vector<int32_t>* pointOrder, const std::vector<int32_t>* subset, int32_t capTotal) {
    const std::string e = buildBoundaries(t, xyz, morton, nThreads, capCells, capPoints, pointOrder, subset, capTotal);
    return e.empty() ? buildTables(t, isInternal, subset != nullptr) : e;
}

std::string SmoothTiles::buildBoundaries(const Topology& t, const double* xyz, bool morton, int32_t nThreads, int32_t capCells,
                                         int32_t capPoints, const std::vector<int32_t>* pointOrder, const std::vector<int32_t>* subset, int32_t capTotal) {
    threads = nThreads;
    PhaseTimer tm(subset ? "shared-point" : "smoothing");
    if (subset) order = *subset;
    else if (morton) order = pointOrder ? *pointOrder : mortonOrder(t.nPoints, xyz);
    else order = naturalOrder(t.nPoints);
    const int32_t nPos = (int32_t)order.size();
    maxCells = maxPoints = 0;
    tm.lap("order");
    const int32_t capTile = threads;
    const auto& pc = t.pointCells;
    const auto& pe = t.pointEdges;
    {
        const int segs = (nPos >= (2 << 20)) ? (int)std::min<unsigned>(hostThreads(), tileSegments()) : 1;
        std::vector<std::vector<int32_t>> segBeg((size_t)segs);
        std::vector<std::string> segErr((size_t)segs);
        parallelRanges(nPos, segs, [&](int sg, int64_t p0, int64_t p1) {
            Stamps stampC((size_t)t.nCells), stampN((size_t)t.nPoints);
            std::vector<int32_t>& beg = segBeg[(size_t)sg];
            int32_t tile = 1, nC = 0, nN = 0, nT = 0;
            for (int32_t pi = (int32_t)p0; pi < (int32_t)p1; ++pi) {
                const int32_t p = order[(size_t)pi];
                for (int attempt = 0; attempt < 2; ++attempt) {
                    int32_t addC = 0, addN = 0;
                    for (int32_t k = pc.off[p]; k < pc.off[p + 1]; ++k)
                        if (stampC[pc.val[k]] != tile) { stampC[pc.val[k]] = tile; ++addC; }
                    if (stampN[p] != tile) { stampN[p] = tile; ++addN; }
                    for (int32_t k = pe.off[p]; k < pe.off[p + 1]; ++k)
                        if (stampN[t.pointPoints[k]] != tile) { stampN[t.pointPoints[k]] = tile; ++addN; }
                    if (nT > 0 && (nT + 1 > capTile || nC + addC > capCells || nN + addN > capPoints || nC + addC + nN + addN > capTotal)) {
                        beg.push_back(pi);
                        ++tile; nC = nN = nT = 0;
                        continue;
                    }
                    if (addC > capCells || addN > capPoints) { segErr[(size_t)sg] = "a single point exceeds the LDS tile capacity"; return; }
                    nC += addC; nN += addN; ++nT;
                    break;
                }
            }
        });
        ptBeg.assign(1, 0);
        for (int sg = 0; sg < segs; ++sg) {
            if (!segErr[(size_t)sg].empty()) return segErr[(size_t)sg];
            if (sg > 0) ptBeg.push_back((int32_t)((int64_t)nPos * sg / segs));
            ptBeg.insert(ptBeg.end(), segBeg[(size_t)sg].begin(), segBeg[(size_t)sg].end());
        }
        ptBeg.push_back(nPos);
        nTiles = (nPos > 0) ? (int32_t)ptBeg.size() - 1 : 0;
        if (nPos == 0) ptBeg.assign(1, 0);
    }
    tm.lap("boundaries");
    return "";
}

std::string SmoothTiles::buildTables(const Topology& t, const uint8_t* isInternal, bool subset) {
    PhaseTimer tm(subset ? "shared-point" : "smoothing");
    const int32_t nPos = (int32_t)order.size();
    const auto& pc = t.pointCells;
    const auto& pe = t.pointEdges;
    selfLoc.assign((size_t)nPos, 0);
    const bool pairs = t.maxPointPoints <= 16;
    struct Part {
        std::vector<int32_t> tcIds, tnIds, nCl, nPt, pcBase, ppBase, pfBase;
        std::vector<uint8_t> pcWidth, ppWidth, pfWidth;
        std::vector<uint16_t> pcEll, ppEll, pairEll, pfEll;
        int32_t maxCells = 0, maxPoints = 0;
        std::string err;
    };
    const int parts = rangeParts(nTiles, 64);
    std::vector<Part> P((size_t)parts);
    const int32_t threadsL = threads;
    parallelRanges(nTiles, parts, [&](int part, int64_t tb, int64_t te) {
        Part& o = P[(size_t)part];
        std::vector<int32_t> cells, pts;
        std::vector<std::pair<int32_t, int32_t>> corners;
        ChainScratch chainScratch;
        for (int32_t ti = (int32_t)tb; ti < (int32_t)te; ++ti) {
            cells.clear(); pts.clear();
            const int32_t pb = ptBeg[ti], pend = ptBeg[ti + 1];
            int32_t wc = 0, wn = 0, wf = 0;
            for (int32_t pi = pb; pi < pend; ++pi) {
                const int32_t p = order[(size_t)pi];
                wf = std::max(wf, 2 * (t.pointFaces.off[p + 1] - t.pointFaces.off[p]));
                wc = std::max(wc, pc.off[p + 1] - pc.off[p]);
                wn = std::max(wn, pe.off[p + 1] - pe.off[p]);
                for (int32_t k = pc.off[p]; k < pc.off[p + 1]; ++k) cells.push_back(pc.val[k]);
                pts.push_back(p);
                for (int32_t k = pe.off[p]; k < pe.off[p + 1]; ++k) pts.push_back(t.pointPoints[k]);
            }
            std::sort(cells.begin(), cells.end());
            cells.erase(std::unique(cells.begin(), cells.end()), cells.end());
            std::sort(pts.begin(), pts.end());
            pts.erase(std::unique(pts.begin(), pts.end()), pts.end());
            wc = roundUp4(wc); wn = roundUp4(wn); wf = roundUp4(wf);
            if ((int32_t)cells.size() > 32766 || (int32_t)pts.size() > 32766 || wc > 252 || wn > 252 || wf > 252) {
                o.err = "tile too large for the 15-bit local index tables";
                return;
            }
            auto locC = [&](int32_t c) { return (int32_t)(std::lower_bound(cells.begin(), cells.end(), c) - cells.begin()); };
            auto locN = [&](int32_t q) { return (int32_t)(std::lower_bound(pts.begin(), pts.end(), q) - pts.begin()); };
            o.tcIds.insert(o.tcIds.end(), cells.begin(), cells.end());
            o.nCl.push_back((int32_t)cells.size());
            o.tnIds.insert(o.tnIds.end(), pts.begin(), pts.end());
            o.nPt.push_back((int32_t)pts.size());
            o.pcBase.push_back((int32_t)o.pcEll.size()); o.pcWidth.push_back((uint8_t)wc);
            o.ppBase.push_back((int32_t)o.ppEll.size()); o.ppWidth.push_back((uint8_t)wn);
            const size_t cbase = o.pcEll.size(), nbase = o.ppEll.size();
            o.pcEll.resize(cbase + (size_t)wc * threadsL, kEllPad);
            o.ppEll.resize(nbase + (size_t)wn * threadsL, kEllPad);
            o.pairEll.resize(nbase + (size_t)wn * threadsL, 0);
            o.pfBase.push_back((int32_t)o.pfEll.size()); o.pfWidth.push_back((uint8_t)wf);
            const size_t fbase = o.pfEll.size();
            o.pfEll.resize(fbase + (size_t)wf * threadsL, kEllPad);
            for (int32_t pi = pb; pi < pend; ++pi) {
                const int32_t p = order[(size_t)pi];
                const int32_t tl = pi - pb;
                selfLoc[(size_t)pi] = (uint16_t)locN(p);
                corners.clear();
                for (int32_t k = t.pointFaces.off[p]; k < t.pointFaces.off[p + 1]; ++k) corners.push_back({t.pfPrev[k], t.pfNext[k]});
                chainCorners(corners, chainScratch);
                for (int32_t j = 0; j < 2 * (int32_t)corners.size(); j += 2) {
                    o.pfEll[fbase + ((size_t)(j / 4) * threadsL + tl) * 4 + (j % 4)] = (uint16_t)locN(corners[(size_t)j / 2].first);
                    o.pfEll[fbase + ((size_t)((j + 1) / 4) * threadsL + tl) * 4 + ((j + 1) % 4)] = (uint16_t)locN(corners[(size_t)j / 2].second);
                }
                for (int32_t k = pc.off[p], j = 0; k < pc.off[p + 1]; ++k, ++j)
                    o.pcEll[cbase + ((size_t)(j / 4) * threadsL + tl) * 4 + (j % 4)] = (uint16_t)locC(pc.val[k]);
                const int32_t b = pe.off[p], v = pe.off[p + 1] - b;
                for (int32_t j = 0; j < v; ++j) {
                    const int32_t q = t.pointPoints[b + j];
                    o.ppEll[nbase + ((size_t)(j / 4) * threadsL + tl) * 4 + (j % 4)] = (uint16_t)(locN(q) | (isInternal[q] ? 0x8000 : 0));
                }
                if (pairs) {
                    for (int32_t i = 0; i < v; ++i) {
                        const int32_t qi = t.pointPoints[b + i];
                        uint16_t mask = 0;
                        for (int32_t j = 0; j < v; ++j) {
                            if (j == i) continue;
                            const int32_t qj = t.pointPoints[b + j];
                            int32_t a = pc.off[qi], ae = pc.off[qi + 1], c = pc.off[qj], ce = pc.off[qj + 1];
                            while (a < ae && c < ce) {
                                if (pc.val[a] == pc.val[c]) { mask |= (uint16_t)(1u << j); break; }
                                if (pc.val[a] < pc.val[c]) ++a; else ++c;
                            }
                        }
                        o.pairEll[nbase + ((size_t)(i / 4) * threadsL + tl) * 4 + (i % 4)] = mask;
                    }
                }
            }
            o.maxCells = std::max(o.maxCells, (int32_t)cells.size());
            o.maxPoints = std::max(o.maxPoints, (int32_t)pts.size());
        }
    });
    tcOff.assign(1, 0); tnOff.assign(1, 0);
    pcBase.clear(); pcWidth.clear(); ppBase.clear(); ppWidth.clear(); pfBase.clear(); pfWidth.clear();
    size_t pcTotal = 0, ppTotal = 0, pfTotal = 0;
    for (Part& o : P) {
        if (!o.err.empty()) return o.err;
        for (int32_t n : o.nCl) tcOff.push_back(tcOff.back() + n);
        for (int32_t n : o.nPt) tnOff.push_back(tnOff.back() + n);
        for (int32_t b : o.pcBase) pcBase.push_back((int32_t)(pcTotal + (size_t)b));
        for (int32_t b : o.ppBase) ppBase.push_back((int32_t)(ppTotal + (size_t)b));
        for (int32_t b : o.pfBase) pfBase.push_back((int32_t)(pfTotal + (size_t)b));
        pcWidth.insert(pcWidth.end(), o.pcWidth.begin(), o.pcWidth.end());
        ppWidth.insert(ppWidth.end(), o.ppWidth.begin(), o.ppWidth.end());
        pfWidth.insert(pfWidth.end(), o.pfWidth.begin(), o.pfWidth.end());
        pcTotal += o.pcEll.size(); ppTotal += o.ppEll.size(); pfTotal += o.pfEll.size();
        maxCells = std::max(maxCells, o.maxCells);
        maxPoints = std::max(maxPoints, o.maxPoints);
    }
    if (pcTotal > 0x7fffffffu || ppTotal > 0x7fffffffu || pfTotal > 0x7fffffffu) return "tile tables exceed int32 addressing";
    {
        std::vector<std::vector<int32_t>> a, b;
        std::vector<std::vector<uint16_t>> c, d, e, f;
        for (Part& o : P) {
            a.push_back(std::move(o.tcIds)); b.push_back(std::move(o.tnIds)); c.push_back(std::move(o.pcEll)); d.push_back(std::move(o.ppEll));
            e.push_back(std::move(o.pairEll)); f.push_back(std::move(o.pfEll));
        }
        concatParts(tcIds, a); concatParts(tnIds, b); concatParts(pcEll, c); concatParts(ppEll, d); concatParts(pairEll, e); concatParts(pfEll, f);
    }
    tm.lap("tables");
    return "";
}

std::string EdgeTiles::build(const Topology& t, const double* xyz, bool morton, int32_t nThreads, int32_t capPoints,
                             int32_t capFaces, int32_t capCells, const std::vector<int32_t>* pointOrder, int32_t capTotal) {
    const std::string e = buildBoundaries(t, xyz, morton, nThreads, capPoints, capFaces, capCells, pointOrder, capTotal);
    return e.empty() ? buildTables(t) : e;
}

std::string EdgeTiles::buildBoundaries(const Topology& t, const double* xyz, bool morton, int32_t nThreads, int32_t capPoints,
                                       int32_t capFaces, int32_t capCells, const std::vector<int32_t>* pointOrder, int32_t capTotal) {
    threads = nThreads;
    PhaseTimer tm("edge");
    const int32_t nE = t.nEdges;
    if (morton && pointOrder) {
        std::vector<int32_t> startOff((size_t)t.nPoints + 1);
        parallelRanges(nE, rangeParts(nE), [&](int, int64_t b, int64_t e1) {
            for (int64_t e = b; e < e1; ++e) {
                const int32_t p = t.edges[2 * e], prev = e > 0 ? t.edges[2 * (e - 1)] : -1;
                for (int32_t q = prev + 1; q <= p; ++q) startOff[(size_t)q] = (int32_t)e;
            }
        });
        for (int32_t q = (nE > 0 ? t.edges[2 * ((size_t)nE - 1)] : -1) + 1; q <= t.nPoints; ++q) startOff[(size_t)q] = nE;
        const std::vector<int32_t>& po = *pointOrder;
        std::vector<int32_t> outOff(po.size() + 1, 0);
        for (size_t i = 0; i < po.size(); ++i) outOff[i + 1] = outOff[i] + (startOff[(size_t)po[i] + 1] - startOff[(size_t)po[i]]);
        resizeHuge(order, (size_t)nE);
        parallelRanges((int64_t)po.size(), rangeParts((int64_t)po.size()), [&](int, int64_t b, int64_t e1) {
            for (int64_t i = b; i < e1; ++i) {
                int32_t o = outOff[(size_t)i];
                for (int32_t e = startOff[(size_t)po[(size_t)i]]; e < startOff[(size_t)po[(size_t)i] + 1]; ++e) order[(size_t)o++] = e;
            }
        });
    } else if (morton) {
        std::vector<double> mid(3 * (size_t)nE);
        parallelRanges(nE, rangeParts(nE), [&](int, int64_t b, int64_t e1) {
            for (int64_t e = b; e < e1; ++e)
                for (int a = 0; a < 3; ++a) mid[3 * (size_t)e + a] = 0.5 * (xyz[3 * (size_t)t.edges[2 * e] + a] + xyz[3 * (size_t)t.edges[2 * e + 1] + a]);
        });
        order = mortonOrder(nE, mid.data());
    } else order = naturalOrder(nE);
    tm.lap("order");
    const auto& ef = t.edgeFaces;
    const auto& ec = t.edgeCells;
    const int segs = (nE >= (4 << 20)) ? (int)std::min<unsigned>(hostThreads(), tileSegments()) : 1;
    std::vector<std::vector<int32_t>> segBeg((size_t)segs);
    std::vector<std::string> segErr((size_t)segs);
    parallelRanges(nE, segs, [&](int sg, int64_t e0, int64_t e1) {
        Stamps stP((size_t)t.nPoints), stF((size_t)t.nFaces), stC((size_t)t.nCells);
        std::vector<int32_t>& beg = segBeg[(size_t)sg];
        int32_t tile = 1, nP = 0, nF = 0, nC = 0, nT = 0;
        for (int32_t ei = (int32_t)e0; ei < (int32_t)e1; ++ei) {
            const int32_t e = order[(size_t)ei];
            for (int attempt = 0; attempt < 2; ++attempt) {
                int32_t aP = 0, aF = 0, aC = 0;
                for (int k = 0; k < 2; ++k) { const int32_t p = t.edges[2 * e + k]; if (stP[p] != tile) { stP[p] = tile; ++aP; } }
                for (int32_t k = ef.off[e]; k < ef.off[e + 1]; ++k) { const int32_t f = ef.val[k]; if (stF[f] != tile) { stF[f] = tile; ++aF; } }
                for (int32_t k = ec.off[e]; k < ec.off[e + 1]; ++k) { const int32_t cI = ec.val[k]; if (stC[cI] != tile) { stC[cI] = tile; ++aC; } }
                if (nT > 0 && (nT + 1 > threads || nP + aP > capPoints || nF + aF > capFaces || nC + aC > capCells || nP + aP + nF + aF + nC + aC > capTotal)) {
                    beg.push_back(ei);
                    ++tile; nP = nF = nC = nT = 0;
                    continue;
                }
                if (aP > capPoints || aF > capFaces || aC > capCells) { segErr[(size_t)sg] = "a single edge exceeds the LDS tile capacity"; return; }
                nP += aP; nF += aF; nC += aC; ++nT;
                break;
            }
        }
    });
    edgeBeg.assign(1, 0);
    for (int sg = 0; sg < segs; ++sg) {
        if (!segErr[(size_t)sg].empty()) return segErr[(size_t)sg];
        if (sg > 0) edgeBeg.push_back((int32_t)((int64_t)nE * sg / segs));
        edgeBeg.insert(edgeBeg.end(), segBeg[(size_t)sg].begin(), segBeg[(size_t)sg].end());
    }
    edgeBeg.push_back(nE);
    nTiles = (int32_t)edgeBeg.size() - 1;
    tm.lap("boundaries");
    return "";
}

std::string EdgeTiles::buildTables(const Topology& t) {
    PhaseTimer tm("edge");
    const int32_t nE = t.nEdges;
    const auto& ef = t.edgeFaces;
    const auto& ec = t.edgeCells;
    epLoc.assign(2 * (size_t)nE, 0);
    struct Part {
        std::vector<int32_t> tpIds, tfIds, tcIds, nP, nF, nC, efBase, ecBase;
        std::vector<uint8_t> efWidth, ecWidth;
        std::vector<uint16_t> efEll, ecEll;
        int32_t maxPoints = 0, maxFaces = 0, maxCells = 0;
        std::string err;
    };
    const int parts = rangeParts(nTiles, 64);
    std::vector<Part> P((size_t)parts);
    const int32_t threadsL = threads;
    parallelRanges(nTiles, parts, [&](int part, int64_t tb, int64_t te) {
        Part& o = P[(size_t)part];
        std::vector<int32_t> pts, fcs, cls;
        for (int32_t ti = (int32_t)tb; ti < (int32_t)te; ++ti) {
            pts.clear(); fcs.clear(); cls.clear();
            const int32_t eb = edgeBeg[ti], ee = edgeBeg[ti + 1];
            int32_t wf = 0, wc = 0;
            for (int32_t ei = eb; ei < ee; ++ei) {
                const int32_t e = order[(size_t)ei];
                wf = std::max(wf, ef.off[e + 1] - ef.off[e]);
                wc = std::max(wc, ec.off[e + 1] - ec.off[e]);
                pts.push_back(t.edges[2 * e]); pts.push_back(t.edges[2 * e + 1]);
                for (int32_t k = ef.off[e]; k < ef.off[e + 1]; ++k) fcs.push_back(ef.val[k]);
                for (int32_t k = ec.off[e]; k < ec.off[e + 1]; ++k) cls.push_back(ec.val[k]);
            }
            std::sort(pts.begin(), pts.end()); pts.erase(std::unique(pts.begin(), pts.end()), pts.end());
            std::sort(fcs.begin(), fcs.end()); fcs.erase(std::unique(fcs.begin(), fcs.end()), fcs.end());
            std::sort(cls.begin(), cls.end()); cls.erase(std::unique(cls.begin(), cls.end()), cls.end());
            wf = roundUp4(wf); wc = roundUp4(wc);
            if (pts.size() > 32766 || fcs.size() > 32766 || cls.size() > 32766 || wf > 252 || wc > 252) {
                o.err = "tile too large for the 15-bit local index tables";
                return;
            }
            auto loc = [](const std::vector<int32_t>& v, int32_t x) { return (int32_t)(std::lower_bound(v.begin(), v.end(), x) - v.begin()); };
            o.tpIds.insert(o.tpIds.end(), pts.begin(), pts.end()); o.nP.push_back((int32_t)pts.size());
            o.tfIds.insert(o.tfIds.end(), fcs.begin(), fcs.end()); o.nF.push_back((int32_t)fcs.size());
            o.tcIds.insert(o.tcIds.end(), cls.begin(), cls.end()); o.nC.push_back((int32_t)cls.size());
            o.efBase.push_back((int32_t)o.efEll.size()); o.efWidth.push_back((uint8_t)wf);
            o.ecBase.push_back((int32_t)o.ecEll.size()); o.ecWidth.push_back((uint8_t)wc);
            const size_t fb = o.efEll.size(), cb = o.ecEll.size();
            o.efEll.resize(fb + (size_t)wf * threadsL, kEllPad);
            o.ecEll.resize(cb + (size_t)wc * threadsL, kEllPad);
            for (int32_t ei = eb; ei < ee; ++ei) {
                const int32_t e = order[(size_t)ei], tl = ei - eb;
                epLoc[2 * (size_t)ei] = (uint16_t)loc(pts, t.edges[2 * e]);
                epLoc[2 * (size_t)ei + 1] = (uint16_t)loc(pts, t.edges[2 * e + 1]);
                if (!t.edgeRingOk[(size_t)e]) continue;
                for (int32_t k = ef.off[e], j = 0; k < ef.off[e + 1]; ++k, ++j)
                    o.efEll[fb + ((size_t)(j / 4) * threadsL + tl) * 4 + (j % 4)] = (uint16_t)loc(fcs, t.ringFace[k]);
                for (int32_t k = ec.off[e], j = 0; k < ec.off[e + 1]; ++k, ++j)
                    o.ecEll[cb + ((size_t)(j / 4) * threadsL + tl) * 4 + (j % 4)] = (uint16_t)loc(cls, t.ringCell[k]);
            }
            o.maxPoints = std::max(o.maxPoints, (int32_t)pts.size());
            o.maxFaces = std::max(o.maxFaces, (int32_t)fcs.size());
            o.maxCells = std::max(o.maxCells, (int32_t)cls.size());
        }
    });
    tpOff.assign(1, 0); tfOff.assign(1, 0); tcOff.assign(1, 0);
    efBase.clear(); ecBase.clear(); efWidth.clear(); ecWidth.clear();
    size_t efTotal = 0, ecTotal = 0;
    for (Part& o : P) {
        if (!o.err.empty()) return o.err;
        for (int32_t n : o.nP) tpOff.push_back(tpOff.back() + n);
        for (int32_t n : o.nF) tfOff.push_back(tfOff.back() + n);
        for (int32_t n : o.nC) tcOff.push_back(tcOff.back() + n);
        for (int32_t b : o.efBase) efBase.push_back((int32_t)(efTotal + (size_t)b));
        for (int32_t b : o.ecBase) ecBase.push_back((int32_t)(ecTotal + (size_t)b));
        efWidth.insert(efWidth.end(), o.efWidth.begin(), o.efWidth.end());
        ecWidth.insert(ecWidth.end(), o.ecWidth.begin(), o.ecWidth.end());
        efTotal += o.efEll.size(); ecTotal += o.ecEll.size();
        maxPoints = std::max(maxPoints, o.maxPoints);
        maxFaces = std::max(maxFaces, o.maxFaces);
        maxCells = std::max(maxCells, o.maxCells);
    }
    if (efTotal > 0x7fffffffu || ecTotal > 0x7fffffffu) return "tile tables exceed int32 addressing";
    {
        std::vector<std::vector<int32_t>> a, b, c;
        std::vector<std::vector<uint16_t>> d, e;
        for (Part& o : P) {
            a.push_back(std::move(o.tpIds)); b.push_back(std::move(o.tfIds)); c.push_back(std::move(o.tcIds));
            d.push_back(std::move(o.efEll)); e.push_back(std::move(o.ecEll));
        }
        concatParts(tpIds, a); concatParts(tfIds, b); concatParts(tcIds, c); concatParts(efEll, d); concatParts(ecEll, e);
    }
    tm.lap("tables");
    return "";
}

}
```

### smoothmesh_amd/csrc/tiles.hpp

```cpp
#pragma once
#include <cstdint>
#include <string>
#include <vector>

#include "topology.hpp"

namespace smgpu {

constexpr uint16_t kEllPad = 0xFFFF;

std::vector<int32_t> mortonOrderOf(int32_t n, const double* xyz);

struct GeomTiles {
    int32_t nTiles = 0, threads = 0;
    std::vector<int32_t> cellBeg;
    std::vector<int32_t> tpOff;
    std::vector<int32_t> tpIds;
    std::vector<int32_t> tfOff;
    std::vector<int32_t> tfIds;
    std::vector<int32_t> fvBase;
    std::vector<uint8_t> fvWidth;
    std::vector<uint16_t> faceVerts;
    std::vector<int32_t> cfBase;
    std::vector<uint8_t> cfWidth;
    std::vector<uint16_t> cellFaces;
    std::vector<uint8_t> tileFlags;
    int32_t maxPoints = 0, maxFaces = 0;
    std::vector<int32_t> order;
    std::string build(const Topology& t, const double* points, bool morton, int32_t threads, int32_t capCells,
                      int32_t capPoints, int32_t capFaces, int32_t capWeighted = 0x7fffffff, int32_t faceWeight = 7);
    std::string buildBoundaries(const Topology& t, const double* points, bool morton, int32_t threads, int32_t capCells,
                                int32_t capPoints, int32_t capFaces, int32_t capWeighted = 0x7fffffff, int32_t faceWeight = 7,
                                const std::vector<int32_t>* cellOrder = nullptr);
    std::string buildTables(const Topology& t);
};
struct GeomTilesDev {
    struct Arr { void* p = nullptr; size_t bytes = 0; };
    Arr cellOrder, cellBeg, tpIds, tfIds, faceVerts, cellFaces, meta;
    bool valid = false;
};
struct DeviceTopologyArrays;
int cellMortonOrderOnDevice(const DeviceTopologyArrays& td, int32_t nCells, int32_t nPoints, const double* points, int device, std::vector<int32_t>& order, std::string& why);
int buildGeomTablesOnDevice(GeomTiles& gt, const DeviceTopologyArrays& td, int32_t nCells, int device, GeomTilesDev& out, std::string& why);

struct SmoothTiles {
    int32_t nTiles = 0, threads = 0;
    std::vector<int32_t> ptBeg;
    std::vector<int32_t> tcOff;
    std::vector<int32_t> tcIds;
    std::vector<int32_t> tnOff;
    std::vector<int32_t> tnIds;
    std::vector<uint16_t> selfLoc;
    std::vector<int32_t> pcBase;
    std::vector<uint8_t> pcWidth;
    std::vector<uint16_t> pcEll;
    std::vector<int32_t> ppBase;
    std::vector<uint8_t> ppWidth;
    std::vector<uint16_t> ppEll;
    std::vector<uint16_t> pairEll;
    std::vector<int32_t> pfBase;
    std::vector<uint8_t> pfWidth;
    std::vector<uint16_t> pfEll;
    int32_t maxCells = 0, maxPoints = 0;
    std::vector<int32_t> order;
    std::string build(const Topology& t, const double* points, const uint8_t* isInternal, bool morton, int32_t threads,
                      int32_t capCells, int32_t capPoints, const std::vector<int32_t>* pointOrder = nullptr,
                      const std::vector<int32_t>* subset = nullptr, int32_t capTotal = 0x7fffffff);
    std::string buildBoundaries(const Topology& t, const double* points, bool morton, int32_t threads, int32_t capCells, int32_t capPoints,
                                const std::vector<int32_t>* pointOrder = nullptr, const std::vector<int32_t>* subset = nullptr, int32_t capTotal = 0x7fffffff);
    std::string buildTables(const Topology& t, const uint8_t* isInternal, bool subset = false);
};
struct SmoothTilesDev {
    struct Arr { void* p = nullptr; size_t bytes = 0; };
    Arr order, ptBeg, tcIds, tnIds, selfLoc, pcEll, ppEll, pairEll, pfEll, meta;
    bool valid = false;
};
struct CornerChains { int* chPrev = nullptr; int* chNext = nullptr; int* bad = nullptr; int* big = nullptr; void* stream = nullptr; int32_t nPoints = 0; bool started = false; };
int startCornerChains(const DeviceTopologyArrays& td, int32_t nPoints, int device, CornerChains& c, std::string& why);
void releaseCornerChains(CornerChains& c);
int buildSmoothTablesOnDevice(SmoothTiles& st, const DeviceTopologyArrays& td, int32_t nPoints, int32_t maxPointPoints, const uint8_t* isInternal, int device,
                              SmoothTilesDev& out, std::string& why, CornerChains* chains = nullptr);

struct EdgeTiles {
    int32_t nTiles = 0, threads = 0;
    std::vector<int32_t> order;
    std::vector<int32_t> edgeBeg;
    std::vector<int32_t> tpOff, tpIds, tfOff, tfIds, tcOff, tcIds;
    std::vector<uint16_t> epLoc;
    std::vector<int32_t> efBase, ecBase;
    std::vector<uint8_t> efWidth, ecWidth;
    std::vector<uint16_t> efEll, ecEll;
    int32_t maxPoints = 0, maxFaces = 0, maxCells = 0;
    std::string build(const Topology& t, const double* points, bool morton, int32_t threads, int32_t capPoints,
                      int32_t capFaces, int32_t capCells, const std::vector<int32_t>* pointOrder = nullptr, int32_t capTotal = 0x7fffffff);
    std::string buildBoundaries(const Topology& t, const double* points, bool morton, int32_t threads, int32_t capPoints,
                                int32_t capFaces, int32_t capCells, const std::vector<int32_t>* pointOrder = nullptr, int32_t capTotal = 0x7fffffff);
    std::string buildTables(const Topology& t);
};
struct EdgeTilesDev {
    struct Arr { void* p = nullptr; size_t bytes = 0; };
    Arr order, edgeBeg, tpIds, tfIds, tcIds, epLoc, efEll, ecEll, meta;
    long long nTf = 0;
    bool valid = false;
};
int buildEdgeTablesOnDevice(EdgeTiles& et, const DeviceTopologyArrays& td, int32_t nEdges, int device, EdgeTilesDev& out, std::string& why);
int remapEdgeFaceIdsOnDevice(const int* geomTfIds, long long nGeomTf, int32_t nFaces, int* edgeTfIds, long long nEdgeTf, int device, std::string& why);

}
```

### smoothmesh_amd/csrc/tiles_dev.hip

```cpp
#include <hip/hip_runtime.h>

#include <cstring>

#include <rocprim/device/device_radix_sort.hpp>
#include <rocprim/device/device_scan.hpp>

#include <algorithm>
#include <chrono>
#include <cstdio>
#include <cstdlib>
#include <string>
#include <vector>

#include "tiles.hpp"

namespace smgpu {

namespace {

constexpr int kT = 256;
constexpr int kBuf = 4096;
constexpr int kPadKey = 0x7fffffff;
typedef unsigned long long u64;

// ... 442 lines not shown
    if ((threadIdx.x & 63) == 0) for (int a = 0; a < 3; ++a) { sh[a][threadIdx.x >> 6] = lo[a]; sh[3 + a][threadIdx.x >> 6] = hi[a]; }
    __syncthreads();
    if (threadIdx.x < 6) {
        double m = sh[threadIdx.x][0];
        for (int i = 1; i < kT / 64; ++i) m = threadIdx.x < 3 ? fmin(m, sh[threadIdx.x][i]) : fmax(m, sh[threadIdx.x][i]);
        part[6 * (size_t)blockIdx.x + threadIdx.x] = m;
    }
}
__device__ __forceinline__ u64 spread21d(u64 v) {
    v &= 0x1fffff;
    v = (v | v << 32) & 0x1f00000000ffffull;
    v = (v | v << 16) & 0x1f0000ff0000ffull;
    v = (v | v << 8) & 0x100f00f00f00f00full;
    v = (v | v << 4) & 0x10c30c30c30c30c3ull;
    v = (v | v << 2) & 0x1249249249249249ull;
    return v;
}
__global__ void __launch_bounds__(kT) k_tl_mortonKeys(int n, const double* __restrict__ xyz, double lo0, double lo1, double lo2, double scale, u64* __restrict__ keys, int* __restrict__ ids) {
    const int i = blockIdx.x * kT + threadIdx.x;
    if (i >= n) return;
    const double lo[3] = {lo0, lo1, lo2};
    u64 k = 0;
    for (int a = 0; a < 3; ++a) k |= spread21d((u64)((xyz[3 * (size_t)i + a] - lo[a]) * scale)) << a;
    keys[i] = k;
    ids[i] = i;
}

struct DevBuf {
    std::vector<void*> all;
    ~DevBuf() { for (void* p : all) (void)hipFree(p); }
    template <class T> T* get(size_t n) {
        void* p = nullptr;
        if (hipMalloc(&p, std::max<size_t>(n, 1) * sizeof(T)) != hipSuccess) { (void)hipGetLastError(); return nullptr; }
        all.push_back(p);
        return (T*)p;
    }
    void release(void* p) { auto it = std::find(all.begin(), all.end(), p); if (it != all.end()) all.erase(it); }
};

}

int buildGeomTablesOnDevice(GeomTiles& gt, const DeviceTopologyArrays& td, int32_t nCells, int device, GeomTilesDev& out, std::string& why) {
    if (!td.valid || !td.owner.p || gt.threads != kT || gt.nTiles <= 0) return 1;
    TL_OK(hipSetDevice(device));
    hipStream_t st = nullptr;
    TL_OK(hipStreamCreateWithFlags(&st, hipStreamNonBlocking));
    struct StreamGuard { hipStream_t s; ~StreamGuard() { (void)hipStreamDestroy(s); } } guard{st};
    const int nT = gt.nTiles;
    DevBuf D;
    int *dOrder = D.get<int>((size_t)nCells), *dBeg = D.get<int>((size_t)nT + 1), *cellTile = D.get<int>((size_t)nCells);
    int *nPts = D.get<int>((size_t)nT), *nFcs = D.get<int>((size_t)nT), *fw = D.get<int>((size_t)nT), *cw = D.get<int>((size_t)nT), *flags = D.get<int>((size_t)nT), *bad = D.get<int>(1);
    long long* terms = D.get<long long>(8 * ((size_t)nT + 1));
    if (!dOrder || !dBeg || !cellTile || !nPts || !nFcs || !fw || !cw || !flags || !bad || !terms) { why = "device allocation failed"; return 2; }
    TL_OK(hipMemcpyAsync(dOrder, gt.order.data(), (size_t)nCells * 4, hipMemcpyHostToDevice, st));
    TL_OK(hipMemcpyAsync(dBeg, gt.cellBeg.data(), ((size_t)nT + 1) * 4, hipMemcpyHostToDevice, st));
    TL_OK(hipMemsetAsync(bad, 0, 4, st));
    GeomIn in{dOrder, dBeg, nT, (const int*)td.cfOff.p, (const int*)td.cfVal.p, (const int*)td.faceOff.p, (const int*)td.facePts.p, (const int*)td.owner.p, cellTile};
    GeomSizes sz{nPts, nFcs, fw, cw, flags, bad};
    hipLaunchKernelGGL(k_tl_cellTile, dim3(nT), dim3(kT), 0, st, in, cellTile);
    hipLaunchKernelGGL(k_tl_geom<false>, dim3(nT), dim3(kT), 0, st, in, sz, GeomOut{});
    long long *tA = terms, *tB = tA + nT + 1, *tC = tB + nT + 1, *tD = tC + nT + 1, *oA = tD + nT + 1, *oB = oA + nT + 1, *oC = oB + nT + 1, *oD = oC + nT + 1;
    TL_OK(hipMemsetAsync(terms, 0, 8 * ((size_t)nT + 1) * 8, st));
    hipLaunchKernelGGL(k_tl_geomTerms, dim3((nT + kT - 1) / kT), dim3(kT), 0, st, nT, sz, tA, tB, tC, tD);
    size_t tempBytes = 0;
    (void)rocprim::exclusive_scan(nullptr, tempBytes, tA, oA, 0ll, (size_t)nT + 1, rocprim::plus<long long>(), st);
    void* temp = D.get<char>(tempBytes + 256);
    if (!temp) { why = "device allocation failed"; return 2; }
    for (int q = 0; q < 4; ++q) {
        size_t b = tempBytes;
        TL_OK(rocprim::exclusive_scan(temp, b, tA + (size_t)q * (nT + 1), oA + (size_t)q * (nT + 1), 0ll, (size_t)nT + 1, rocprim::plus<long long>(), st));
    }
    std::vector<long long> offs(4 * ((size_t)nT + 1));
    int hbad = 0;
    TL_OK(hipMemcpyAsync(offs.data(), oA, offs.size() * 8, hipMemcpyDeviceToHost, st));
    TL_OK(hipMemcpyAsync(&hbad, bad, 4, hipMemcpyDeviceToHost, st));
    TL_OK(hipStreamSynchronize(st));
    if (hbad) return 1;
    const long long nTp = offs[(size_t)nT], nTf = offs[(size_t)(nT + 1) + nT], nFv = offs[2 * (size_t)(nT + 1) + nT], nCf = offs[3 * (size_t)(nT + 1) + nT];
    if (nTp > 0x7fffffffll || nTf > 0x7fffffffll || nFv > 0x7fffffffll || nCf > 0x7fffffffll) return 1;
    int *tpIds = D.get<int>((size_t)nTp), *tfIds = D.get<int>((size_t)nTf), *meta = D.get<int>(12 * (size_t)nT);
    uint16_t *faceVerts = D.get<uint16_t>((size_t)nFv), *cellFaces = D.get<uint16_t>((size_t)nCf);
    if (!tpIds || !tfIds || !meta || !faceVerts || !cellFaces) { why = "device allocation failed"; return 2; }
    TL_OK(hipMemsetAsync(cellFaces, 0xFF, (size_t)nCf * 2, st));
    hipLaunchKernelGGL(k_tl_geom<true>, dim3(nT), dim3(kT), 0, st, in, sz, GeomOut{oA, oB, oC, oD, tpIds, tfIds, faceVerts, cellFaces, meta});
    std::vector<int> hN((size_t)nT), hF((size_t)nT), hFw((size_t)nT), hCw((size_t)nT), hFl((size_t)nT);
    gt.tfIds.resize((size_t)nTf);
    TL_OK(hipMemcpyAsync(hN.data(), nPts, (size_t)nT * 4, hipMemcpyDeviceToHost, st));
    TL_OK(hipMemcpyAsync(hF.data(), nFcs, (size_t)nT * 4, hipMemcpyDeviceToHost, st));
    TL_OK(hipMemcpyAsync(hFw.data(), fw, (size_t)nT * 4, hipMemcpyDeviceToHost, st));
    TL_OK(hipMemcpyAsync(hCw.data(), cw, (size_t)nT * 4, hipMemcpyDeviceToHost, st));
    TL_OK(hipMemcpyAsync(hFl.data(), flags, (size_t)nT * 4, hipMemcpyDeviceToHost, st));
    TL_OK(hipMemcpyAsync(gt.tfIds.data(), tfIds, (size_t)nTf * 4, hipMemcpyDeviceToHost, st));
    TL_OK(hipStreamSynchronize(st));
    TL_OK(hipGetLastError());
    gt.tpOff.resize((size_t)nT + 1); gt.tfOff.resize((size_t)nT + 1); gt.fvBase.resize((size_t)nT); gt.cfBase.resize((size_t)nT);
    gt.fvWidth.resize((size_t)nT); gt.cfWidth.resize((size_t)nT); gt.tileFlags.resize((size_t)nT);
    gt.maxPoints = gt.maxFaces = 0;
    for (int i = 0; i <= nT; ++i) { gt.tpOff[(size_t)i] = (int32_t)offs[(size_t)i]; gt.tfOff[(size_t)i] = (int32_t)offs[(size_t)(nT + 1) + i]; }
    for (int i = 0; i < nT; ++i) {
        gt.fvBase[(size_t)i] = (int32_t)offs[2 * (size_t)(nT + 1) + i]; gt.cfBase[(size_t)i] = (int32_t)offs[3 * (size_t)(nT + 1) + i];
        gt.fvWidth[(size_t)i] = (uint8_t)hFw[(size_t)i]; gt.cfWidth[(size_t)i] = (uint8_t)hCw[(size_t)i]; gt.tileFlags[(size_t)i] = (uint8_t)hFl[(size_t)i];
        gt.maxPoints = std::max(gt.maxPoints, hN[(size_t)i]); gt.maxFaces = std::max(gt.maxFaces, hF[(size_t)i]);
    }
    gt.tpIds.clear(); gt.faceVerts.clear(); gt.cellFaces.clear();
    auto give = [&](GeomTilesDev::Arr& a, void* p, size_t bytes) { a.p = p; a.bytes = std::max<size_t>(bytes, 1); D.release(p); };
    give(out.cellOrder, dOrder, (size_t)nCells * 4); give(out.cellBeg, dBeg, ((size_t)nT + 1) * 4);
    give(out.tpIds, tpIds, (size_t)nTp * 4); give(out.tfIds, tfIds, (size_t)nTf * 4);
    give(out.faceVerts, faceVerts, (size_t)nFv * 2); give(out.cellFaces, cellFaces, (size_t)nCf * 2); give(out.meta, meta, 12 * (size_t)nT * 4);
    out.valid = true;
    return 0;
}

int buildEdgeTablesOnDevice(EdgeTiles& et, const DeviceTopologyArrays& td, int32_t nEdges, int device, EdgeTilesDev& out, std::string& why) {
    if (!td.valid || et.threads != kT || et.nTiles <= 0) return 1;
    TL_OK(hipSetDevice(device));
    hipStream_t st = nullptr;
    TL_OK(hipStreamCreateWithFlags(&st, hipStreamNonBlocking));
    struct StreamGuard { hipStream_t s; ~StreamGuard() { (void)hipStreamDestroy(s); } } guard{st};
    const int nT = et.nTiles;
    DevBuf D;
    int *dOrder = D.get<int>((size_t)nEdges), *dBeg = D.get<int>((size_t)nT + 1);
    int *nPts = D.get<int>((size_t)nT), *nFcs = D.get<int>((size_t)nT), *nCls = D.get<int>((size_t)nT), *wf = D.get<int>((size_t)nT), *wc = D.get<int>((size_t)nT), *bad = D.get<int>(1);
    long long* terms = D.get<long long>(10 * ((size_t)nT + 1));
    if (!dOrder || !dBeg || !nPts || !nFcs || !nCls || !wf || !wc || !bad || !terms) { why = "device allocation failed"; return 2; }
    TL_OK(hipMemcpyAsync(dOrder, et.order.data(), (size_t)nEdges * 4, hipMemcpyHostToDevice, st));
    TL_OK(hipMemcpyAsync(dBeg, et.edgeBeg.data(), ((size_t)nT + 1) * 4, hipMemcpyHostToDevice, st));
    TL_OK(hipMemsetAsync(bad, 0, 4, st));
    EdgeIn in{dOrder, dBeg, nT, (const int*)td.edges.p, (const int*)td.efOff.p, (const int*)td.efFace.p, (const int*)td.ecOff.p, (const int*)td.ecCell.p,
              (const int*)td.ringFace.p, (const int*)td.ringCell.p, (const uint8_t*)td.edgeRingOk.p};
    EdgeSizes sz{nPts, nFcs, nCls, wf, wc, bad};
    hipLaunchKernelGGL(k_tl_edge<false>, dim3(nT), dim3(kT), 0, st, in, sz, EdgeOut{});
    const size_t S = (size_t)nT + 1;
    TL_OK(hipMemsetAsync(terms, 0, 10 * S * 8, st));
    hipLaunchKernelGGL(k_tl_edgeTerms, dim3((nT + kT - 1) / kT), dim3(kT), 0, st, nT, sz, terms, terms + S, terms + 2 * S, terms + 3 * S, terms + 4 * S);
    long long* offsD = terms + 5 * S;
    size_t tempBytes = 0;
    (void)rocprim::exclusive_scan(nullptr, tempBytes, terms, offsD, 0ll, S, rocprim::plus<long long>(), st);
    void* temp = D.get<char>(tempBytes + 256);
    if (!temp) { why = "device allocation failed"; return 2; }
    for (int q = 0; q < 5; ++q) { size_t b = tempBytes; TL_OK(rocprim::exclusive_scan(temp, b, terms + (size_t)q * S, offsD + (size_t)q * S, 0ll, S, rocprim::plus<long long>(), st)); }
    std::vector<long long> offs(5 * S);
    int hbad = 0;
    TL_OK(hipMemcpyAsync(offs.data(), offsD, offs.size() * 8, hipMemcpyDeviceToHost, st));
    TL_OK(hipMemcpyAsync(&hbad, bad, 4, hipMemcpyDeviceToHost, st));
    TL_OK(hipStreamSynchronize(st));
    if (hbad) return 1;
    const long long nTp = offs[(size_t)nT], nTf = offs[S + nT], nTc = offs[2 * S + nT], nEf = offs[3 * S + nT], nEc = offs[4 * S + nT];
    if (nTp > 0x7fffffffll || nTf > 0x7fffffffll || nTc > 0x7fffffffll || nEf > 0x7fffffffll || nEc > 0x7fffffffll) return 1;
    int *tpIds = D.get<int>((size_t)nTp), *tfIds = D.get<int>((size_t)nTf), *tcIds = D.get<int>((size_t)nTc), *meta = D.get<int>(12 * (size_t)nT);
    uint16_t *epLoc = D.get<uint16_t>(2 * (size_t)nEdges), *efEll = D.get<uint16_t>((size_t)nEf), *ecEll = D.get<uint16_t>((size_t)nEc);
    if (!tpIds || !tfIds || !tcIds || !meta || !epLoc || !efEll || !ecEll) { why = "device allocation failed"; return 2; }
    TL_OK(hipMemsetAsync(efEll, 0xFF, (size_t)nEf * 2, st));
    TL_OK(hipMemsetAsync(ecEll, 0xFF, (size_t)nEc * 2, st));
    TL_OK(hipMemsetAsync(epLoc, 0, 2 * (size_t)nEdges * 2, st));
    hipLaunchKernelGGL(k_tl_edge<true>, dim3(nT), dim3(kT), 0, st, in, sz, EdgeOut{offsD, offsD + S, offsD + 2 * S, offsD + 3 * S, offsD + 4 * S, tpIds, tfIds, tcIds, epLoc, efEll, ecEll, meta});
    std::vector<int> hP((size_t)nT), hF((size_t)nT), hC((size_t)nT), hWf((size_t)nT), hWc((size_t)nT);
    TL_OK(hipMemcpyAsync(hP.data(), nPts, (size_t)nT * 4, hipMemcpyDeviceToHost, st));
    TL_OK(hipMemcpyAsync(hF.data(), nFcs, (size_t)nT * 4, hipMemcpyDeviceToHost, st));
    TL_OK(hipMemcpyAsync(hC.data(), nCls, (size_t)nT * 4, hipMemcpyDeviceToHost, st));
    TL_OK(hipMemcpyAsync(hWf.data(), wf, (size_t)nT * 4, hipMemcpyDeviceToHost, st));
    TL_OK(hipMemcpyAsync(hWc.data(), wc, (size_t)nT * 4, hipMemcpyDeviceToHost, st));
    TL_OK(hipStreamSynchronize(st));
    TL_OK(hipGetLastError());
    et.tpOff.resize(S); et.tfOff.resize(S); et.tcOff.resize(S); et.efBase.resize((size_t)nT); et.ecBase.resize((size_t)nT); et.efWidth.resize((size_t)nT); et.ecWidth.resize((size_t)nT);
    et.maxPoints = et.maxFaces = et.maxCells = 0;
    for (size_t i = 0; i < S; ++i) { et.tpOff[i] = (int32_t)offs[i]; et.tfOff[i] = (int32_t)offs[S + i]; et.tcOff[i] = (int32_t)offs[2 * S + i]; }
    for (int i = 0; i < nT; ++i) {
        et.efBase[(size_t)i] = (int32_t)offs[3 * S + i]; et.ecBase[(size_t)i] = (int32_t)offs[4 * S + i];
        et.efWidth[(size_t)i] = (uint8_t)hWf[(size_t)i]; et.ecWidth[(size_t)i] = (uint8_t)hWc[(size_t)i];
        et.maxPoints = std::max(et.maxPoints, hP[(size_t)i]); et.maxFaces = std::max(et.maxFaces, hF[(size_t)i]); et.maxCells = std::max(et.maxCells, hC[(size_t)i]);
    }
    et.tpIds.clear(); et.tfIds.clear(); et.tcIds.clear(); et.epLoc.clear(); et.efEll.clear(); et.ecEll.clear();
    auto give = [&](EdgeTilesDev::Arr& a, void* p, size_t bytes) { a.p = p; a.bytes = std::max<size_t>(bytes, 1); D.release(p); };
    give(out.order, dOrder, (size_t)nEdges * 4); give(out.edgeBeg, dBeg, S * 4);
    give(out.tpIds, tpIds, (size_t)nTp * 4); give(out.tfIds, tfIds, (size_t)nTf * 4); give(out.tcIds, tcIds, (size_t)nTc * 4);
    give(out.epLoc, epLoc, 2 * (size_t)nEdges * 2); give(out.efEll, efEll, (size_t)nEf * 2); give(out.ecEll, ecEll, (size_t)nEc * 2); give(out.meta, meta, 12 * (size_t)nT * 4);
    out.nTf = nTf;
    out.valid = true;
    return 0;
}

int startCornerChains(const DeviceTopologyArrays& td, int32_t nPoints, int device, CornerChains& c, std::string& why) {
    if (!td.valid || nPoints <= 0) return 1;
    TL_OK(hipSetDevice(device));
    const size_t nPf = td.pfPrev.bytes / 4;
    hipStream_t st = nullptr;
    TL_OK(hipStreamCreateWithFlags(&st, hipStreamNonBlocking));
    int *a = nullptr, *b = nullptr, *bad = nullptr, *big = nullptr;
    if (hipMalloc((void**)&a, std::max<size_t>(nPf, 1) * 4) != hipSuccess || hipMalloc((void**)&b, std::max<size_t>(nPf, 1) * 4) != hipSuccess || hipMalloc((void**)&bad, 4) != hipSuccess ||
        hipMalloc((void**)&big, ((size_t)nPoints + 1) * 4) != hipSuccess) {
        (void)hipGetLastError();
        if (a) (void)hipFree(a);
        if (b) (void)hipFree(b);
        if (bad) (void)hipFree(bad);
        (void)hipStreamDestroy(st);
        why = "device allocation failed";
        return 2;
    }
    c.chPrev = a; c.chNext = b; c.bad = bad; c.big = big; c.stream = (void*)st; c.nPoints = nPoints;
    (void)hipMemsetAsync(bad, 0, 4, st);
    launchChains(st, nPoints, nullptr, (const int*)td.pfOff.p, (const int*)td.pfPrev.p, (const int*)td.pfNext.p, a, b, big, bad);
    c.started = true;
    return 0;
}
void releaseCornerChains(CornerChains& c) {
    if (!c.started) return;
    (void)hipStreamSynchronize((hipStream_t)c.stream);
    (void)hipStreamDestroy((hipStream_t)c.stream);
    (void)hipFree(c.chPrev); (void)hipFree(c.chNext); (void)hipFree(c.bad);
    if (c.big) (void)hipFree(c.big);
    c = CornerChains();
}

int buildSmoothTablesOnDevice(SmoothTiles& st, const DeviceTopologyArrays& td, int32_t nPoints, int32_t maxPointPoints, const uint8_t* isInternal, int device,
                              SmoothTilesDev& out, std::string& why, CornerChains* chains) {
    struct ChainGuard { CornerChains* c; ~ChainGuard() { if (c) releaseCornerChains(*c); } } chainGuard{chains};
    if (!td.valid || st.threads != kT || st.nTiles <= 0 || st.order.empty()) return 1;
    const bool haveChains = chains && chains->started && chains->nPoints == nPoints;
    const int nPos = (int)st.order.size();
    TL_OK(hipSetDevice(device));
    hipStream_t sm = nullptr;
    TL_OK(hipStreamCreateWithFlags(&sm, hipStreamNonBlocking));
    struct StreamGuard { hipStream_t s; ~StreamGuard() { (void)hipStreamDestroy(s); } } guard{sm};
    const int nT = st.nTiles;
    const size_t S = (size_t)nT + 1, nPf = td.pfPrev.bytes / 4;
    DevBuf D;
    int *dOrder = D.get<int>((size_t)nPos), *dBeg = D.get<int>(S);
    int *chPrev = haveChains ? chains->chPrev : D.get<int>(nPf), *chNext = haveChains ? chains->chNext : D.get<int>(nPf);
    uint8_t* dInt = D.get<uint8_t>((size_t)nPoints);
    int *nCl = D.get<int>((size_t)nT), *nPt = D.get<int>((size_t)nT), *wc = D.get<int>((size_t)nT), *wn = D.get<int>((size_t)nT), *wf = D.get<int>((size_t)nT), *bad = D.get<int>(1);
    long long* terms = D.get<long long>(10 * S);
    if (!dOrder || !dBeg || !chPrev || !chNext || !dInt || !nCl || !nPt || !wc || !wn || !wf || !bad || !terms) { why = "device allocation failed"; return 2; }
    TL_OK(hipMemsetAsync(bad, 0, 4, sm));
    TL_OK(hipMemcpyAsync(dOrder, st.order.data(), (size_t)nPos * 4, hipMemcpyHostToDevice, sm));
    if (haveChains) {
        TL_OK(hipStreamSynchronize((hipStream_t)chains->stream));
        int cb = 0;
        TL_OK(hipMemcpy(&cb, chains->bad, 4, hipMemcpyDeviceToHost));
        if (cb) return 1;
    } else {
        int* big = D.get<int>((size_t)nPos + 1);
        if (!big) { why = "device allocation failed"; return 2; }
        launchChains(sm, nPos, nPos == nPoints ? (const int*)nullptr : (const int*)dOrder, (const int*)td.pfOff.p, (const int*)td.pfPrev.p, (const int*)td.pfNext.p, chPrev, chNext, big, bad);
    }
    TL_OK(hipMemcpyAsync(dBeg, st.ptBeg.data(), S * 4, hipMemcpyHostToDevice, sm));
    TL_OK(hipMemcpyAsync(dInt, isInternal, (size_t)nPoints, hipMemcpyHostToDevice, sm));
    SmoothIn in{dOrder, dBeg, nT, maxPointPoints <= 16 ? 1 : 0, (const int*)td.pcOff.p, (const int*)td.pcVal.p, (const int*)td.ppOff.p, (const int*)td.ppPt.p,
                (const int*)td.pfOff.p, chPrev, chNext, dInt};
    SmoothSizes sz{nCl, nPt, wc, wn, wf, bad};
    hipLaunchKernelGGL(k_tl_smooth<false>, dim3(nT), dim3(kT), 0, sm, in, sz, SmoothOut{});
    TL_OK(hipMemsetAsync(terms, 0, 10 * S * 8, sm));
    hipLaunchKernelGGL(k_tl_smoothTerms, dim3((nT + kT - 1) / kT), dim3(kT), 0, sm, nT, sz, terms, terms + S, terms + 2 * S, terms + 3 * S, terms + 4 * S);
    long long* offsD = terms + 5 * S;
    size_t tempBytes = 0;
    (void)rocprim::exclusive_scan(nullptr, tempBytes, terms, offsD, 0ll, S, rocprim::plus<long long>(), sm);
    void* temp = D.get<char>(tempBytes + 256);
    if (!temp) { why = "device allocation failed"; return 2; }
    for (int q = 0; q < 5; ++q) { size_t b = tempBytes; TL_OK(rocprim::exclusive_scan(temp, b, terms + (size_t)q * S, offsD + (size_t)q * S, 0ll, S, rocprim::plus<long long>(), sm)); }
    std::vector<long long> offs(5 * S);
    int hbad = 0;
    TL_OK(hipMemcpyAsync(offs.data(), offsD, offs.size() * 8, hipMemcpyDeviceToHost, sm));
    TL_OK(hipMemcpyAsync(&hbad, bad, 4, hipMemcpyDeviceToHost, sm));
    TL_OK(hipStreamSynchronize(sm));
    if (hbad) return 1;
    const long long nTc = offs[(size_t)nT], nTn = offs[S + nT], nPc = offs[2 * S + nT], nPp = offs[3 * S + nT], nPfE = offs[4 * S + nT];
    if (nTc > 0x7fffffffll || nTn > 0x7fffffffll || nPc > 0x7fffffffll || nPp > 0x7fffffffll || nPfE > 0x7fffffffll) return 1;
    int *tcIds = D.get<int>((size_t)nTc), *tnIds = D.get<int>((size_t)nTn), *meta = D.get<int>(12 * (size_t)nT);
    uint16_t *selfLoc = D.get<uint16_t>((size_t)nPos), *pcEll = D.get<uint16_t>((size_t)nPc), *ppEll = D.get<uint16_t>((size_t)nPp), *pairEll = D.get<uint16_t>((size_t)nPp),
             *pfEll = D.get<uint16_t>((size_t)nPfE);
    if (!tcIds || !tnIds || !meta || !selfLoc || !pcEll || !ppEll || !pairEll || !pfEll) { why = "device allocation failed"; return 2; }
    TL_OK(hipMemsetAsync(pcEll, 0xFF, (size_t)nPc * 2, sm));
    TL_OK(hipMemsetAsync(ppEll, 0xFF, (size_t)nPp * 2, sm));
    TL_OK(hipMemsetAsync(pfEll, 0xFF, (size_t)nPfE * 2, sm));
    TL_OK(hipMemsetAsync(pairEll, 0, (size_t)nPp * 2, sm));
    TL_OK(hipMemsetAsync(selfLoc, 0, (size_t)nPos * 2, sm));
    hipLaunchKernelGGL(k_tl_smooth<true>, dim3(nT), dim3(kT), 0, sm, in, sz,
                       SmoothOut{offsD, offsD + S, offsD + 2 * S, offsD + 3 * S, offsD + 4 * S, tcIds, tnIds, selfLoc, pcEll, ppEll, pairEll, pfEll, meta});
    std::vector<int> hC((size_t)nT), hN((size_t)nT), hWc((size_t)nT), hWn((size_t)nT), hWf((size_t)nT);
    TL_OK(hipMemcpyAsync(hC.data(), nCl, (size_t)nT * 4, hipMemcpyDeviceToHost, sm));
    TL_OK(hipMemcpyAsync(hN.data(), nPt, (size_t)nT * 4, hipMemcpyDeviceToHost, sm));
    TL_OK(hipMemcpyAsync(hWc.data(), wc, (size_t)nT * 4, hipMemcpyDeviceToHost, sm));
    TL_OK(hipMemcpyAsync(hWn.data(), wn, (size_t)nT * 4, hipMemcpyDeviceToHost, sm));
    TL_OK(hipMemcpyAsync(hWf.data(), wf, (size_t)nT * 4, hipMemcpyDeviceToHost, sm));
    TL_OK(hipStreamSynchronize(sm));
    TL_OK(hipGetLastError());
    st.tcOff.resize(S); st.tnOff.resize(S);
    st.pcBase.resize((size_t)nT); st.ppBase.resize((size_t)nT); st.pfBase.resize((size_t)nT); st.pcWidth.resize((size_t)nT); st.ppWidth.resize((size_t)nT); st.pfWidth.resize((size_t)nT);
    st.maxCells = st.maxPoints = 0;
    for (size_t i = 0; i < S; ++i) { st.tcOff[i] = (int32_t)offs[i]; st.tnOff[i] = (int32_t)offs[S + i]; }
    for (int i = 0; i < nT; ++i) {
        st.pcBase[(size_t)i] = (int32_t)offs[2 * S + i]; st.ppBase[(size_t)i] = (int32_t)offs[3 * S + i]; st.pfBase[(size_t)i] = (int32_t)offs[4 * S + i];
        st.pcWidth[(size_t)i] = (uint8_t)hWc[(size_t)i]; st.ppWidth[(size_t)i] = (uint8_t)hWn[(size_t)i]; st.pfWidth[(size_t)i] = (uint8_t)hWf[(size_t)i];
        st.maxCells = std::max(st.maxCells, hC[(size_t)i]); st.maxPoints = std::max(st.maxPoints, hN[(size_t)i]);
    }
    st.tcIds.clear(); st.tnIds.clear(); st.selfLoc.clear(); st.pcEll.clear(); st.ppEll.clear(); st.pairEll.clear(); st.pfEll.clear();
    auto give = [&](SmoothTilesDev::Arr& a, void* p, size_t bytes) { a.p = p; a.bytes = std::max<size_t>(bytes, 1); D.release(p); };
    give(out.order, dOrder, (size_t)nPos * 4); give(out.ptBeg, dBeg, S * 4); give(out.tcIds, tcIds, (size_t)nTc * 4); give(out.tnIds, tnIds, (size_t)nTn * 4);
    give(out.selfLoc, selfLoc, (size_t)nPos * 2); give(out.pcEll, pcEll, (size_t)nPc * 2); give(out.ppEll, ppEll, (size_t)nPp * 2); give(out.pairEll, pairEll, (size_t)nPp * 2);
    give(out.pfEll, pfEll, (size_t)nPfE * 2); give(out.meta, meta, 12 * (size_t)nT * 4);
    out.valid = true;
    return 0;
}

int cellMortonOrderOnDevice(const DeviceTopologyArrays& td, int32_t nCells, int32_t nPoints, const double* points, int device, std::vector<int32_t>& order, std::string& why) {
    if (!td.valid || nCells <= 0 || nPoints <= 0) return 1;
    TL_OK(hipSetDevice(device));
    hipStream_t st = nullptr;
    TL_OK(hipStreamCreateWithFlags(&st, hipStreamNonBlocking));
    struct StreamGuard { hipStream_t s; ~StreamGuard() { (void)hipStreamDestroy(s); } } guard{st};
    const int nB = (nCells + kT - 1) / kT;
    DevBuf D;
    double *dPts = D.get<double>(3 * (size_t)nPoints), *cc = D.get<double>(3 * (size_t)nCells), *part = D.get<double>(6 * (size_t)nB);
    u64 *kA = D.get<u64>((size_t)nCells), *kB = D.get<u64>((size_t)nCells);
    int *iA = D.get<int>((size_t)nCells), *iB = D.get<int>((size_t)nCells);
    if (!dPts || !cc || !part || !kA || !kB || !iA || !iB) { why = "device allocation failed"; return 2; }
    TL_OK(hipMemcpyAsync(dPts, points, 3 * (size_t)nPoints * 8, hipMemcpyHostToDevice, st));
    hipLaunchKernelGGL(k_tl_cellAvg, dim3(nB), dim3(kT), 0, st, nCells, (const int*)td.cfOff.p, (const int*)td.cfVal.p, (const int*)td.faceOff.p, (const int*)td.facePts.p, dPts, cc, part);
    std::vector<double> hp(6 * (size_t)nB);
    TL_OK(hipMemcpyAsync(hp.data(), part, hp.size() * 8, hipMemcpyDeviceToHost, st));
    TL_OK(hipStreamSynchronize(st));
    double lo[3] = {1e300, 1e300, 1e300}, hi[3] = {-1e300, -1e300, -1e300};
    for (int b = 0; b < nB; ++b)
        for (int a = 0; a < 3; ++a) { lo[a] = std::min(lo[a], hp[6 * (size_t)b + a]); hi[a] = std::max(hi[a], hp[6 * (size_t)b + 3 + a]); }
    double ext = 0.0;
    for (int a = 0; a < 3; ++a) ext = std::max(ext, hi[a] - lo[a]);
    const double scale = ext > 0.0 ? 2097151.0 / ext : 0.0;
    hipLaunchKernelGGL(k_tl_mortonKeys, dim3(nB), dim3(kT), 0, st, nCells, cc, lo[0], lo[1], lo[2], scale, kA, iA);
    size_t tempBytes = 0;
    (void)rocprim::radix_sort_pairs(nullptr, tempBytes, kA, kB, iA, iB, (size_t)nCells, 0, 63, st);
    void* temp = D.get<char>(tempBytes + 256);
    if (!temp) { why = "device allocation failed"; return 2; }
    TL_OK(rocprim::radix_sort_pairs(temp, tempBytes, kA, kB, iA, iB, (size_t)nCells, 0, 63, st));
    order.resize((size_t)nCells);
    TL_OK(hipMemcpyAsync(order.data(), iB, (size_t)nCells * 4, hipMemcpyDeviceToHost, st));
    TL_OK(hipStreamSynchronize(st));
    TL_OK(hipGetLastError());
    return 0;
}

int remapEdgeFaceIdsOnDevice(const int* geomTfIds, long long nGeomTf, int32_t nFaces, int* edgeTfIds, long long nEdgeTf, int device, std::string& why) {
    TL_OK(hipSetDevice(device));
    int* facePos = nullptr;
    TL_OK(hipMalloc((void**)&facePos, std::max<size_t>((size_t)nFaces, 1) * 4));
    struct Free { int* p; ~Free() { (void)hipFree(p); } } guard{facePos};
    TL_OK(hipMemset(facePos, 0xFF, (size_t)nFaces * 4));
    hipLaunchKernelGGL(k_tl_facePos, dim3((unsigned)((nGeomTf + kT - 1) / kT)), dim3(kT), 0, nullptr, nGeomTf, geomTfIds, facePos);
    hipLaunchKernelGGL(k_tl_remap, dim3((unsigned)((nEdgeTf + kT - 1) / kT)), dim3(kT), 0, nullptr, nEdgeTf, edgeTfIds, facePos);
    TL_OK(hipDeviceSynchronize());
    TL_OK(hipGetLastError());
    return 0;
}

}
```

Measured before the change: 12.25 billion.

## Align Morton keys to mesh lattice and deduplicate identical tile index blocks

Adds a lattice-aligned Morton frame, enabled by default for all-hex meshes, so that tiles over a regular mesh get identical local connectivity. It then hashes and compares the per-tile ELL index blocks on the host or device and points tile metadata at one shared representative block. The aim is a smaller working set of connectivity tables streamed each iteration, so more of it stays in cache and less HBM traffic goes to index data. It adds setup work (hashing, pairwise compares, extra uploads), and the benefit depends on the mesh being regular.

```diff
diff --git a/smoothmesh_amd/csrc/smgpu.hip b/smoothmesh_amd/csrc/smgpu.hip
--- a/smoothmesh_amd/csrc/smgpu.hip
+++ b/smoothmesh_amd/csrc/smgpu.hip
@@ -480,8 +480,11 @@
     auto sinceCreate = [&] { return std::chrono::duration<double>(std::chrono::steady_clock::now() - tCreate0).count(); };
     const bool wantTiles = envInt("SMGPU_TILES", 1) != 0;
     const bool mortonTiles = envInt("SMGPU_TILE_MORTON", 1) != 0;
+    const bool allHex = tileLatticeDefault(d->nCells, d->nFaces, d->nInternalFaces, d->nFaces > 0 ? (int64_t)d->faceOffsets[d->nFaces] - d->faceOffsets[0] : 0);
+    const bool latticeKeys = tileLatticeKnob(allHex);
+    h->gt.latticeKeys = h->stl.latticeKeys = h->etl.latticeKeys = latticeKeys;
     std::future<std::vector<int32_t>> fPointOrder;
-    if (wantTiles && mortonTiles) fPointOrder = std::async(std::launch::async, [&] { return mortonOrderOf(d->nPoints, d->points); });
+    if (wantTiles && mortonTiles) fPointOrder = std::async(std::launch::async, [&] { return mortonOrderOf(d->nPoints, d->points, latticeKeys); });
     std::future<std::string> fGeom, fSmooth, fEdge;
     std::function<void()> startEdge;
     CornerChains chains;
@@ -506,7 +509,7 @@
                       std::vector<int32_t> cellOrder;
                       if (mortonTiles && devTiles && devTopo.valid && envInt("SMGPU_DEVICE_TILES", 1) == 1) {
                           std::string why;
-                          if (cellMortonOrderOnDevice(devTopo, d->nCells, d->nPoints, d->points, h->device, cellOrder, why) != 0) cellOrder.clear();
+                          if (cellMortonOrderOnDevice(devTopo, d->nCells, d->nPoints, d->points, h->device, cellOrder, why, latticeKeys) != 0) cellOrder.clear();
                       }
                       const std::string e = h->gt.buildBoundaries(h->topo, d->points, mortonTiles, geomT0, geomCells0, capGP0, capGF0,
                                                                   envInt("SMGPU_GEOM_CAPWEIGHTED", defaultGeomCapWeighted(geomT0)), SMGPU_GEOM_AOS ? kGF : 6,
@@ -750,17 +753,42 @@
             rc |= devUpload(h, &g.cfBase, h->gt.cfBase);
             rc |= devUpload(h, &g.cfWidth, h->gt.cfWidth);
             rc |= devUpload(h, &g.tileFlags, h->gt.tileFlags);
-            if (!g.meta) {
+            const bool shareTiles = tileShareKnob();
+            auto shareDev = [&](TileShare& out, int nT, const uint16_t* a, const uint16_t* b, const std::vector<int32_t>& base, auto lenOf, const std::vector<uint8_t>& width) {
+                std::vector<int32_t> len((size_t)nT), key(width.begin(), width.end());
+                for (int t = 0; t < nT; ++t) len[(size_t)t] = (int32_t)lenOf(t);
+                std::string why;
+                if (shareBlocksOnDevice(nT, a, b, base, len, key, h->device, out, why)) rc |= fail("smgpu_create: shared tile blocks: " + why);
+            };
+            auto putMeta = [&](const int*& dst, const std::vector<int>& meta) {
+                if (!dst) { rc |= devUpload(h, &dst, meta); return; }
+                if (!meta.empty() && hipMemcpy((void*)dst, meta.data(), meta.size() * sizeof(int), hipMemcpyHostToDevice) != hipSuccess) rc |= fail("smgpu_create: upload of the tile records failed");
+            };
+            const bool sayTiles = envInt("SMGPU_VERBOSE", 0) != 0;
+            int dFv = h->gt.nTiles, dCf = h->gt.nTiles, dPc = h->stl.nTiles, dPp = h->stl.nTiles, dPf = h->stl.nTiles;
+            if (!g.meta || shareTiles) {
                 const auto& gt = h->gt;
+                const int nT = gt.nTiles;
+                TileShare fv, cf;
+                if (gt.faceVerts.empty() && g.faceVerts) {
+                    shareDev(fv, nT, g.faceVerts, nullptr, gt.fvBase, [&](int t) { return (size_t)(gt.tfOff[(size_t)t + 1] - gt.tfOff[(size_t)t]) * gt.fvWidth[(size_t)t]; }, gt.fvWidth);
+                    shareDev(cf, nT, g.cellFaces, nullptr, gt.cfBase, [&](int t) { return (size_t)gt.cfWidth[(size_t)t] * (size_t)gt.threads; }, gt.cfWidth);
+                } else shareGeomBlocks(gt, gt.faceVerts.data(), gt.cellFaces.data(), fv, cf);
+                if (rc) return cleanup(1);
                 std::vector<int> meta((size_t)kGeomMetaInts * (size_t)gt.nTiles, 0);
                 for (int t = 0; t < gt.nTiles; ++t) {
                     int* r = meta.data() + (size_t)kGeomMetaInts * t;
                     r[0] = gt.tpOff[t]; r[1] = gt.tpOff[t + 1] - gt.tpOff[t]; r[2] = gt.tfOff[t]; r[3] = gt.tfOff[t + 1] - gt.tfOff[t];
-                    r[4] = gt.fvBase[t]; r[5] = gt.fvWidth[t]; r[6] = gt.cellBeg[t]; r[7] = gt.cellBeg[t + 1] - gt.cellBeg[t];
-                    r[8] = gt.cfBase[t]; r[9] = gt.cfWidth[t]; r[10] = gt.tileFlags[t];
+                    r[4] = fv.remap(gt.fvBase, t); r[5] = gt.fvWidth[t]; r[6] = gt.cellBeg[t]; r[7] = gt.cellBeg[t + 1] - gt.cellBeg[t];
+                    r[8] = cf.remap(gt.cfBase, t); r[9] = gt.cfWidth[t]; r[10] = gt.tileFlags[t];
                 }
-                rc |= devUpload(h, &g.meta, meta);
+                putMeta(g.meta, meta);
+                dFv = fv.distinct; dCf = cf.distinct;
             }
+            if (sayTiles)
+                std::fprintf(stderr, "[smgpu] geometry tiles: %d tiles, distinct blocks: faceVerts %d, cellFaces %d (SMGPU_TILE_LATTICE=%d SMGPU_TILE_SHARE=%d), staged faces x%.4f, "
+                             "staged points x%.4f\n", h->gt.nTiles, dFv, dCf, (int)h->gt.latticeKeys, (int)shareTiles, (double)h->gt.tfOff.back() / std::max(1, t.nFaces),
+                             (double)h->gt.tpOff.back() / std::max(1, t.nPoints));
             g.maxPoints = h->gt.maxPoints; g.maxFaces = h->gt.maxFaces;
             if (h->stDev.valid) {
                 auto adoptS = [&](auto*& dst, const SmoothTilesDev::Arr& a) { dst = (std::remove_reference_t<decltype(dst)>)a.p; h->allocs.push_back(a.p); h->deviceBytes += (int64_t)a.bytes; };
@@ -786,17 +814,30 @@
             rc |= devUpload(h, &v.ppWidth, h->stl.ppWidth);
             rc |= devUpload(h, &v.pfBase, h->stl.pfBase);
             rc |= devUpload(h, &v.pfWidth, h->stl.pfWidth);
-            if (!v.meta) {
+            if (!v.meta || shareTiles) {
                 const auto& st = h->stl;
+                const int nS = st.nTiles;
+                TileShare pc, pp, pf;
+                if (st.pcEll.empty() && v.pcEll) {
+                    const size_t T = (size_t)st.threads;
+                    shareDev(pc, nS, v.pcEll, nullptr, st.pcBase, [&](int t) { return st.pcWidth[(size_t)t] * T; }, st.pcWidth);
+                    shareDev(pp, nS, v.ppEll, v.pairEll, st.ppBase, [&](int t) { return st.ppWidth[(size_t)t] * T; }, st.ppWidth);
+                    shareDev(pf, nS, v.pfEll, nullptr, st.pfBase, [&](int t) { return st.pfWidth[(size_t)t] * T; }, st.pfWidth);
+                } else shareSmoothBlocks(st, st.pcEll.data(), st.ppEll.data(), st.pairEll.data(), st.pfEll.data(), pc, pp, pf);
+                if (rc) return cleanup(1);
                 std::vector<int> meta((size_t)kSmoothMetaInts * (size_t)st.nTiles, 0);
                 for (int t = 0; t < st.nTiles; ++t) {
                     int* r = meta.data() + (size_t)kSmoothMetaInts * t;
                     r[0] = st.ptBeg[t]; r[1] = st.ptBeg[t + 1] - st.ptBeg[t]; r[2] = st.tcOff[t]; r[3] = st.tcOff[t + 1] - st.tcOff[t];
-                    r[4] = st.tnOff[t]; r[5] = st.tnOff[t + 1] - st.tnOff[t]; r[6] = st.pcBase[t]; r[7] = st.pcWidth[t];
-                    r[8] = st.ppBase[t]; r[9] = st.ppWidth[t]; r[10] = st.pfBase[t]; r[11] = st.pfWidth[t];
+                    r[4] = st.tnOff[t]; r[5] = st.tnOff[t + 1] - st.tnOff[t]; r[6] = pc.remap(st.pcBase, t); r[7] = st.pcWidth[t];
+                    r[8] = pp.remap(st.ppBase, t); r[9] = st.ppWidth[t]; r[10] = pf.remap(st.pfBase, t); r[11] = st.pfWidth[t];
                 }
-                rc |= devUpload(h, &v.meta, meta);
+                putMeta(v.meta, meta);
+                dPc = pc.distinct; dPp = pp.distinct; dPf = pf.distinct;
             }
+            if (sayTiles)
+                std::fprintf(stderr, "[smgpu] smoothing tiles: %d tiles, distinct blocks: pcEll %d, ppEll+pairEll %d, pfEll %d, staged cell centres x%.4f, staged points x%.4f (per point)\n",
+                             h->stl.nTiles, dPc, dPp, dPf, (double)h->stl.tcOff.back() / std::max(1, t.nPoints), (double)h->stl.tnOff.back() / std::max(1, t.nPoints));
             v.maxCells = h->stl.maxCells; v.maxPoints = h->stl.maxPoints;
             v.usePairShare = t.maxPointPoints <= 16 ? 1 : 0;
             if (h->useFilter) {
@@ -838,17 +879,30 @@
                     rc |= devUpload(h, &ev.ecBase, h->etl.ecBase);
                     rc |= devUpload(h, &ev.efWidth, h->etl.efWidth);
                     rc |= devUpload(h, &ev.ecWidth, h->etl.ecWidth);
-                    if (!ev.meta) {
+                    int dEf = h->etl.nTiles, dEc = h->etl.nTiles;
+                    if (!ev.meta || shareTiles) {
                         const auto& et = h->etl;
+                        const int nE = et.nTiles;
+                        TileShare ef, ec;
+                        if (et.efEll.empty() && ev.efEll) {
+                            const size_t T = (size_t)et.threads;
+                            shareDev(ef, nE, ev.efEll, nullptr, et.efBase, [&](int ti) { return et.efWidth[(size_t)ti] * T; }, et.efWidth);
+                            shareDev(ec, nE, ev.ecEll, nullptr, et.ecBase, [&](int ti) { return et.ecWidth[(size_t)ti] * T; }, et.ecWidth);
+                        } else shareEdgeBlocks(et, et.efEll.data(), et.ecEll.data(), ef, ec);
+                        if (rc) return cleanup(1);
+                        dEf = ef.distinct; dEc = ec.distinct;
                         std::vector<int> meta((size_t)kEdgeMetaInts * (size_t)et.nTiles, 0);
                         for (int ti = 0; ti < et.nTiles; ++ti) {
                             int* r = meta.data() + (size_t)kEdgeMetaInts * ti;
                             r[0] = et.edgeBeg[ti]; r[1] = et.edgeBeg[ti + 1] - et.edgeBeg[ti]; r[2] = et.tpOff[ti]; r[3] = et.tpOff[ti + 1] - et.tpOff[ti];
                             r[4] = et.tfOff[ti]; r[5] = et.tfOff[ti + 1] - et.tfOff[ti]; r[6] = et.tcOff[ti]; r[7] = et.tcOff[ti + 1] - et.tcOff[ti];
-                            r[8] = et.efBase[ti]; r[9] = et.efWidth[ti]; r[10] = et.ecBase[ti]; r[11] = et.ecWidth[ti];
+                            r[8] = ef.remap(et.efBase, ti); r[9] = et.efWidth[ti]; r[10] = ec.remap(et.ecBase, ti); r[11] = et.ecWidth[ti];
                         }
-                        rc |= devUpload(h, &ev.meta, meta);
+                        putMeta(ev.meta, meta);
                     }
+                    if (sayTiles)
+                        std::fprintf(stderr, "[smgpu] edge tiles: %d tiles, distinct blocks: efEll %d, ecEll %d, staged points x%.4f, faces x%.4f, cells x%.4f (per edge)\n", h->etl.nTiles, dEf, dEc,
+                                     (double)h->etl.tpOff.back() / std::max(1, t.nEdges), (double)h->etl.tfOff.back() / std::max(1, t.nEdges), (double)h->etl.tcOff.back() / std::max(1, t.nEdges));
                     ev.maxPoints = h->etl.maxPoints; ev.maxFaces = h->etl.maxFaces; ev.maxCells = h->etl.maxCells;
                     h->edgeLds = sizeof(double) * 3 * maxTileTotal(h->etl.nTiles, {&h->etl.tpOff, &h->etl.tfOff, &h->etl.tcOff});
                     h->edgeTilesOk = h->edgeLds <= 64 * 1024;
diff --git a/smoothmesh_amd/csrc/tiles.cpp b/smoothmesh_amd/csrc/tiles.cpp
--- a/smoothmesh_amd/csrc/tiles.cpp
+++ b/smoothmesh_amd/csrc/tiles.cpp
@@ -35,7 +35,7 @@
     return v;
 }
 
-static std::vector<int32_t> mortonOrder(int32_t n, const double* xyz) {
+static std::vector<int32_t> mortonOrder(int32_t n, const double* xyz, bool lattice) {
     double lo[3] = {1e300, 1e300, 1e300}, hi[3] = {-1e300, -1e300, -1e300};
     {
         const int parts = rangeParts(n);
@@ -49,9 +49,9 @@
         for (int part = 0; part < parts; ++part)
             for (int a = 0; a < 3; ++a) { lo[a] = std::min(lo[a], plo[3 * (size_t)part + a]); hi[a] = std::max(hi[a], phi[3 * (size_t)part + a]); }
     }
-    double ext = 0.0;
-    for (int a = 0; a < 3; ++a) ext = std::max(ext, hi[a] - lo[a]);
-    const double scale = ext > 0.0 ? 2097151.0 / ext : 0.0;
+    const MortonFrame fr = mortonFrame(n, lo, hi, lattice);
+    const double scale = fr.scale;
+    for (int a = 0; a < 3; ++a) lo[a] = fr.origin[a];
     std::vector<std::pair<uint64_t, int32_t>> key((size_t)n);
     parallelRanges(n, rangeParts(n), [&](int, int64_t b, int64_t e) {
         for (int64_t i = b; i < e; ++i) {
@@ -61,7 +61,7 @@
         }
     });
     if (rangeParts(n) > 1) {
-        const int shift = 55;
+        const int shift = std::max(3 * fr.bits - 8, 0);
         std::vector<size_t> cnt(257, 0);
         for (int32_t i = 0; i < n; ++i) ++cnt[(size_t)(key[(size_t)i].first >> shift) + 1];
         for (int bkt = 0; bkt < 256; ++bkt) cnt[(size_t)bkt + 1] += cnt[(size_t)bkt];
@@ -81,7 +81,7 @@
     return order;
 }
 
-std::vector<int32_t> mortonOrderOf(int32_t n, const double* xyz) { return mortonOrder(n, xyz); }
+std::vector<int32_t> mortonOrderOf(int32_t n, const double* xyz, bool lattice) { return mortonOrder(n, xyz, lattice); }
 
 static std::vector<int32_t> naturalOrder(int32_t n) {
     std::vector<int32_t> o((size_t)n);
@@ -136,7 +136,7 @@
                 for (int a = 0; a < 3; ++a) cc[3 * (size_t)c + a] = n ? s[a] / n : 0.0;
             }
         });
-        order = mortonOrder(t.nCells, cc.data());
+        order = mortonOrder(t.nCells, cc.data(), latticeKeys);
     } else order = naturalOrder(t.nCells);
     tm.lap("order");
     {
@@ -285,6 +285,104 @@
 }
 
 namespace {
+struct BlockSpan { const uint16_t* p; size_t n; };
+template <class F> void shareBlocks(int32_t nTiles, TileShare& out, F block) {
+    out.rep.resize((size_t)nTiles);
+    for (int32_t t = 0; t < nTiles; ++t) out.rep[(size_t)t] = t;
+    out.distinct = nTiles;
+    if (!tileShareKnob() || nTiles < 2) return;
+    std::vector<uint64_t> hash((size_t)nTiles);
+    parallelRanges(nTiles, rangeParts(nTiles, 64), [&](int, int64_t tb, int64_t te) {
+        BlockSpan sp[4];
+        for (int32_t t = (int32_t)tb; t < (int32_t)te; ++t) {
+            uint64_t key = 0;
+            const int ns = block(t, sp, key);
+            uint64_t hh = 1469598103934665603ull ^ key;
+            for (int s = 0; s < ns; ++s) {
+                hh = (hh ^ sp[s].n) * 1099511628211ull;
+                for (size_t i = 0; i < sp[s].n; ++i) { hh ^= sp[s].p[i]; hh *= 1099511628211ull; }
+            }
+            hash[(size_t)t] = hh;
+        }
+    });
+    std::vector<int32_t> idx((size_t)nTiles);
+    for (int32_t t = 0; t < nTiles; ++t) idx[(size_t)t] = t;
+    std::sort(idx.begin(), idx.end(), [&](int32_t a, int32_t b) { return hash[(size_t)a] != hash[(size_t)b] ? hash[(size_t)a] < hash[(size_t)b] : a < b; });
+    auto same = [&](int32_t a, int32_t b) {
+        BlockSpan x[4], y[4];
+        uint64_t kx = 0, ky = 0;
+        const int nx = block(a, x, kx), ny = block(b, y, ky);
+        if (nx != ny || kx != ky) return false;
+        for (int s = 0; s < nx; ++s)
+            if (x[s].n != y[s].n || !std::equal(x[s].p, x[s].p + x[s].n, y[s].p)) return false;
+        return true;
+    };
+    std::vector<int32_t> firsts;
+    for (size_t i = 0; i < idx.size();) {
+        size_t j = i;
+        firsts.clear();
+        for (; j < idx.size() && hash[(size_t)idx[j]] == hash[(size_t)idx[i]]; ++j) {
+            const int32_t t = idx[j];
+            bool found = false;
+            for (int32_t f : firsts)
+                if (same(f, t)) { out.rep[(size_t)t] = f; --out.distinct; found = true; break; }
+            if (!found) firsts.push_back(t);
+        }
+        i = j;
+    }
+}
+}
+
+void shareGeomBlocks(const GeomTiles& gt, const uint16_t* faceVerts, const uint16_t* cellFaces, TileShare& fv, TileShare& cf) {
+    shareBlocks(gt.nTiles, fv, [&](int32_t t, BlockSpan* sp, uint64_t& key) {
+        const int32_t nf = gt.tfOff[(size_t)t + 1] - gt.tfOff[(size_t)t];
+        key = gt.fvWidth[(size_t)t];
+        sp[0] = {faceVerts + gt.fvBase[(size_t)t], (size_t)nf * gt.fvWidth[(size_t)t]};
+        return 1;
+    });
+    shareBlocks(gt.nTiles, cf, [&](int32_t t, BlockSpan* sp, uint64_t& key) {
+        key = gt.cfWidth[(size_t)t];
+        sp[0] = {cellFaces + gt.cfBase[(size_t)t], (size_t)gt.cfWidth[(size_t)t] * (size_t)gt.threads};
+        return 1;
+    });
+}
+
+void shareSmoothBlocks(const SmoothTiles& st, const uint16_t* pcEll, const uint16_t* ppEll, const uint16_t* pairEll, const uint16_t* pfEll,
+                       TileShare& pc, TileShare& pp, TileShare& pf) {
+    const size_t T = (size_t)st.threads;
+    shareBlocks(st.nTiles, pc, [&](int32_t t, BlockSpan* sp, uint64_t& key) {
+        key = st.pcWidth[(size_t)t];
+        sp[0] = {pcEll + st.pcBase[(size_t)t], st.pcWidth[(size_t)t] * T};
+        return 1;
+    });
+    shareBlocks(st.nTiles, pp, [&](int32_t t, BlockSpan* sp, uint64_t& key) {
+        key = st.ppWidth[(size_t)t];
+        sp[0] = {ppEll + st.ppBase[(size_t)t], st.ppWidth[(size_t)t] * T};
+        sp[1] = {pairEll + st.ppBase[(size_t)t], st.ppWidth[(size_t)t] * T};
+        return 2;
+    });
+    shareBlocks(st.nTiles, pf, [&](int32_t t, BlockSpan* sp, uint64_t& key) {
+        key = st.pfWidth[(size_t)t];
+        sp[0] = {pfEll + st.pfBase[(size_t)t], st.pfWidth[(size_t)t] * T};
+        return 1;
+    });
+}
+
+void shareEdgeBlocks(const EdgeTiles& et, const uint16_t* efEll, const uint16_t* ecEll, TileShare& ef, TileShare& ec) {
+    const size_t T = (size_t)et.threads;
+    shareBlocks(et.nTiles, ef, [&](int32_t t, BlockSpan* sp, uint64_t& key) {
+        key = et.efWidth[(size_t)t];
+        sp[0] = {efEll + et.efBase[(size_t)t], et.efWidth[(size_t)t] * T};
+        return 1;
+    });
+    shareBlocks(et.nTiles, ec, [&](int32_t t, BlockSpan* sp, uint64_t& key) {
+        key = et.ecWidth[(size_t)t];
+        sp[0] = {ecEll + et.ecBase[(size_t)t], et.ecWidth[(size_t)t] * T};
+        return 1;
+    });
+}
+
+namespace {
 struct ChainScratch {
     std::vector<int32_t> verts, deg, adjOff, adjEdge, ea, eb, stackV, stackE, next;
     std::vector<uint8_t> used;
@@ -365,7 +463,7 @@
     threads = nThreads;
     PhaseTimer tm(subset ? "shared-point" : "smoothing");
     if (subset) order = *subset;
-    else if (morton) order = pointOrder ? *pointOrder : mortonOrder(t.nPoints, xyz);
+    else if (morton) order = pointOrder ? *pointOrder : mortonOrder(t.nPoints, xyz, latticeKeys);
     else order = naturalOrder(t.nPoints);
     const int32_t nPos = (int32_t)order.size();
     maxCells = maxPoints = 0;
@@ -580,7 +678,7 @@
             for (int64_t e = b; e < e1; ++e)
                 for (int a = 0; a < 3; ++a) mid[3 * (size_t)e + a] = 0.5 * (xyz[3 * (size_t)t.edges[2 * e] + a] + xyz[3 * (size_t)t.edges[2 * e + 1] + a]);
         });
-        order = mortonOrder(nE, mid.data());
+        order = mortonOrder(nE, mid.data(), latticeKeys);
     } else order = naturalOrder(nE);
     tm.lap("order");
     const auto& ef = t.edgeFaces;
diff --git a/smoothmesh_amd/csrc/tiles.hpp b/smoothmesh_amd/csrc/tiles.hpp
--- a/smoothmesh_amd/csrc/tiles.hpp
+++ b/smoothmesh_amd/csrc/tiles.hpp
@@ -1,5 +1,8 @@
 #pragma once
+#include <algorithm>
+#include <cmath>
 #include <cstdint>
+#include <cstdlib>
 #include <string>
 #include <vector>
 
@@ -9,10 +12,55 @@
 
 constexpr uint16_t kEllPad = 0xFFFF;
 
-std::vector<int32_t> mortonOrderOf(int32_t n, const double* xyz);
+struct MortonFrame { double origin[3]; double scale; int bits; bool lattice; };
+inline bool tileLatticeKnob(bool dflt = true) { const char* e = std::getenv("SMGPU_TILE_LATTICE"); return e ? std::atoi(e) != 0 : dflt; }
+inline bool tileLatticeDefault(int64_t nCells, int64_t nFaces, int64_t nInternalFaces, int64_t nFacePoints) {
+    return nFaces > 0 && nFacePoints == 4 * nFaces && nFaces + nInternalFaces == 6 * nCells;
+}
+inline MortonFrame mortonFrame(int64_t n, const double lo[3], const double hi[3], bool lattice) {
+    MortonFrame f{{lo[0], lo[1], lo[2]}, 0.0, 21, false};
+    double ext = 0.0, e[3];
+    for (int a = 0; a < 3; ++a) { e[a] = hi[a] - lo[a]; ext = std::max(ext, e[a]); }
+    f.scale = ext > 0.0 ? 2097151.0 / ext : 0.0;
+    if (!lattice || n < 2 || !(ext > 0.0) || !std::isfinite(ext)) return f;
+    int k = 0;
+    double h = 1.0;
+    for (int a = 0; a < 3; ++a) if (e[a] > 0.0) { h *= e[a]; ++k; }
+    h = std::pow(h / (double)n, 1.0 / k);
+    for (int it = 0; it < 16; ++it) {
+        double v = 1.0;
+        for (int a = 0; a < 3; ++a) if (e[a] > 0.0) v *= e[a] + h;
+        h = std::pow(v / (double)n, 1.0 / k);
+    }
+    if (!(h > 0.0) || !std::isfinite(h) || !std::isfinite(1.0 / h) || !(ext / h + 1.0 < 2097151.0)) return f;
+    f.lattice = true;
+    f.scale = 1.0 / h;
+    for (int a = 0; a < 3; ++a) f.origin[a] = lo[a] - 0.5 * h;
+    const uint64_t top = (uint64_t)((ext + 0.5 * h) * f.scale) + 1;
+    f.bits = 1;
+    while (f.bits < 21 && (top >> f.bits)) ++f.bits;
+    return f;
+}
+
+std::vector<int32_t> mortonOrderOf(int32_t n, const double* xyz, bool lattice = tileLatticeKnob());
+
+struct TileShare {
+    std::vector<int32_t> rep;
+    int32_t distinct = 0;
+    int32_t remap(const std::vector<int32_t>& base, int32_t t) const { return base[(size_t)rep[(size_t)t]]; }
+};
+inline bool tileShareKnob() { const char* e = std::getenv("SMGPU_TILE_SHARE"); return !e || std::atoi(e) != 0; }
+struct GeomTiles; struct SmoothTiles; struct EdgeTiles;
+void shareGeomBlocks(const GeomTiles& gt, const uint16_t* faceVerts, const uint16_t* cellFaces, TileShare& fv, TileShare& cf);
+void shareSmoothBlocks(const SmoothTiles& st, const uint16_t* pcEll, const uint16_t* ppEll, const uint16_t* pairEll, const uint16_t* pfEll,
+                       TileShare& pc, TileShare& pp, TileShare& pf);
+void shareEdgeBlocks(const EdgeTiles& et, const uint16_t* efEll, const uint16_t* ecEll, TileShare& ef, TileShare& ec);
+int shareBlocksOnDevice(int32_t nTiles, const uint16_t* a, const uint16_t* b, const std::vector<int32_t>& base, const std::vector<int32_t>& len, const std::vector<int32_t>& key,
+                        int device, TileShare& out, std::string& why);
 
 struct GeomTiles {
     int32_t nTiles = 0, threads = 0;
+    bool latticeKeys = tileLatticeKnob();
     std::vector<int32_t> cellBeg;
     std::vector<int32_t> tpOff;
     std::vector<int32_t> tpIds;
@@ -40,11 +88,13 @@
     bool valid = false;
 };
 struct DeviceTopologyArrays;
-int cellMortonOrderOnDevice(const DeviceTopologyArrays& td, int32_t nCells, int32_t nPoints, const double* points, int device, std::vector<int32_t>& order, std::string& why);
+int cellMortonOrderOnDevice(const DeviceTopologyArrays& td, int32_t nCells, int32_t nPoints, const double* points, int device, std::vector<int32_t>& order, std::string& why,
+                            bool lattice = tileLatticeKnob());
 int buildGeomTablesOnDevice(GeomTiles& gt, const DeviceTopologyArrays& td, int32_t nCells, int device, GeomTilesDev& out, std::string& why);
 
 struct SmoothTiles {
     int32_t nTiles = 0, threads = 0;
+    bool latticeKeys = tileLatticeKnob();
     std::vector<int32_t> ptBeg;
     std::vector<int32_t> tcOff;
     std::vector<int32_t> tcIds;
@@ -83,6 +133,7 @@
 
 struct EdgeTiles {
     int32_t nTiles = 0, threads = 0;
+    bool latticeKeys = tileLatticeKnob();
     std::vector<int32_t> order;
     std::vector<int32_t> edgeBeg;
     std::vector<int32_t> tpOff, tpIds, tfOff, tfIds, tcOff, tcIds;
diff --git a/smoothmesh_amd/csrc/tiles_dev.hip b/smoothmesh_amd/csrc/tiles_dev.hip
--- a/smoothmesh_amd/csrc/tiles_dev.hip
+++ b/smoothmesh_amd/csrc/tiles_dev.hip
@@ -768,7 +768,8 @@
     return 0;
 }
 
-int cellMortonOrderOnDevice(const DeviceTopologyArrays& td, int32_t nCells, int32_t nPoints, const double* points, int device, std::vector<int32_t>& order, std::string& why) {
+int cellMortonOrderOnDevice(const DeviceTopologyArrays& td, int32_t nCells, int32_t nPoints, const double* points, int device, std::vector<int32_t>& order, std::string& why,
+                            bool lattice) {
     if (!td.valid || nCells <= 0 || nPoints <= 0) return 1;
     TL_OK(hipSetDevice(device));
     hipStream_t st = nullptr;
@@ -788,10 +789,8 @@
     double lo[3] = {1e300, 1e300, 1e300}, hi[3] = {-1e300, -1e300, -1e300};
     for (int b = 0; b < nB; ++b)
         for (int a = 0; a < 3; ++a) { lo[a] = std::min(lo[a], hp[6 * (size_t)b + a]); hi[a] = std::max(hi[a], hp[6 * (size_t)b + 3 + a]); }
-    double ext = 0.0;
-    for (int a = 0; a < 3; ++a) ext = std::max(ext, hi[a] - lo[a]);
-    const double scale = ext > 0.0 ? 2097151.0 / ext : 0.0;
-    hipLaunchKernelGGL(k_tl_mortonKeys, dim3(nB), dim3(kT), 0, st, nCells, cc, lo[0], lo[1], lo[2], scale, kA, iA);
+    const MortonFrame fr = mortonFrame(nCells, lo, hi, lattice);
+    hipLaunchKernelGGL(k_tl_mortonKeys, dim3(nB), dim3(kT), 0, st, nCells, cc, fr.origin[0], fr.origin[1], fr.origin[2], fr.scale, kA, iA);
     size_t tempBytes = 0;
     (void)rocprim::radix_sort_pairs(nullptr, tempBytes, kA, kB, iA, iB, (size_t)nCells, 0, 63, st);
     void* temp = D.get<char>(tempBytes + 256);
@@ -801,6 +800,106 @@
     TL_OK(hipMemcpyAsync(order.data(), iB, (size_t)nCells * 4, hipMemcpyDeviceToHost, st));
     TL_OK(hipStreamSynchronize(st));
     TL_OK(hipGetLastError());
+    return 0;
+}
+
+namespace {
+__global__ void __launch_bounds__(kT) k_tl_blockHash(const uint16_t* __restrict__ a, const uint16_t* __restrict__ b, const long long* __restrict__ base, const int* __restrict__ len,
+                                                     u64* __restrict__ hash) {
+    const int t = blockIdx.x;
+    const long long o = base[t];
+    const int n = len[t];
+    u64 h = 0;
+    for (int i = threadIdx.x; i < n; i += kT) {
+        u64 x = ((u64)(unsigned)i << 32) | ((u64)a[o + i] << 16) | (b ? (u64)b[o + i] : 0ull);
+        x *= 0x9E3779B97F4A7C15ull; x ^= x >> 29; x *= 0xBF58476D1CE4E5B9ull; x ^= x >> 32;
+        h += x;
+    }
+    for (int d = 32; d > 0; d >>= 1) h += __shfl_xor(h, d, 64);
+    __shared__ u64 sh[kT / 64];
+    if ((threadIdx.x & 63) == 0) sh[threadIdx.x >> 6] = h;
+    __syncthreads();
+    if (threadIdx.x == 0) {
+        u64 s = 0;
+        for (int i = 0; i < kT / 64; ++i) s += sh[i];
+        hash[t] = s;
+    }
+}
+__global__ void __launch_bounds__(kT) k_tl_blockDiffers(const uint16_t* __restrict__ a, const uint16_t* __restrict__ b, const long long* __restrict__ base, const int* __restrict__ len,
+                                                        const int* __restrict__ pairT, const int* __restrict__ pairR, int* __restrict__ differs) {
+    const int t = pairT[blockIdx.x], r = pairR[blockIdx.x];
+    const long long ot = base[t], orr = base[r];
+    const int n = len[t];
+    bool d = false;
+    for (int i = threadIdx.x; i < n; i += kT) {
+        d |= a[ot + i] != a[orr + i];
+        if (b) d |= b[ot + i] != b[orr + i];
+    }
+    if (d) differs[blockIdx.x] = 1;
+}
+}
+
+int shareBlocksOnDevice(int32_t nTiles, const uint16_t* a, const uint16_t* b, const std::vector<int32_t>& base, const std::vector<int32_t>& len, const std::vector<int32_t>& key, int device,
+                        TileShare& out, std::string& why) {
+    out.rep.resize((size_t)nTiles);
+    for (int32_t t = 0; t < nTiles; ++t) out.rep[(size_t)t] = t;
+    out.distinct = nTiles;
+    if (!tileShareKnob() || nTiles < 2) return 0;
+    TL_OK(hipSetDevice(device));
+    DevBuf D;
+    long long* dBase = D.get<long long>((size_t)nTiles);
+    int* dLen = D.get<int>((size_t)nTiles);
+    u64* dHash = D.get<u64>((size_t)nTiles);
+    if (!dBase || !dLen || !dHash) { why = "device allocation failed"; return 2; }
+    std::vector<long long> hBase(base.begin(), base.end());
+    TL_OK(hipMemcpy(dBase, hBase.data(), (size_t)nTiles * 8, hipMemcpyHostToDevice));
+    TL_OK(hipMemcpy(dLen, len.data(), (size_t)nTiles * 4, hipMemcpyHostToDevice));
+    hipLaunchKernelGGL(k_tl_blockHash, dim3(nTiles), dim3(kT), 0, nullptr, a, b, dBase, dLen, dHash);
+    TL_OK(hipGetLastError());
+    std::vector<u64> hash((size_t)nTiles);
+    TL_OK(hipMemcpy(hash.data(), dHash, (size_t)nTiles * 8, hipMemcpyDeviceToHost));
+    std::vector<int32_t> idx((size_t)nTiles);
+    for (int32_t t = 0; t < nTiles; ++t) idx[(size_t)t] = t;
+    auto groupLess = [&](int32_t x, int32_t y) {
+        if (hash[(size_t)x] != hash[(size_t)y]) return hash[(size_t)x] < hash[(size_t)y];
+        if (len[(size_t)x] != len[(size_t)y]) return len[(size_t)x] < len[(size_t)y];
+        return key[(size_t)x] < key[(size_t)y];
+    };
+    std::sort(idx.begin(), idx.end(), [&](int32_t x, int32_t y) { return groupLess(x, y) || (!groupLess(y, x) && x < y); });
+    std::vector<std::vector<int32_t>> groups;
+    for (size_t i = 0; i < idx.size();) {
+        size_t j = i + 1;
+        while (j < idx.size() && !groupLess(idx[i], idx[j])) ++j;
+        if (j - i > 1) groups.emplace_back(idx.begin() + (std::ptrdiff_t)i, idx.begin() + (std::ptrdiff_t)j);
+        i = j;
+    }
+    std::vector<int> pairT, pairR, differs;
+    while (!groups.empty()) {
+        pairT.clear(); pairR.clear();
+        for (const auto& g : groups)
+            for (size_t k = 1; k < g.size(); ++k) { pairT.push_back(g[k]); pairR.push_back(g[0]); }
+        const size_t nP = pairT.size();
+        int *dT = D.get<int>(nP), *dR = D.get<int>(nP), *dDiff = D.get<int>(nP);
+        if (!dT || !dR || !dDiff) { why = "device allocation failed"; return 2; }
+        TL_OK(hipMemcpy(dT, pairT.data(), nP * 4, hipMemcpyHostToDevice));
+        TL_OK(hipMemcpy(dR, pairR.data(), nP * 4, hipMemcpyHostToDevice));
+        TL_OK(hipMemset(dDiff, 0, nP * 4));
+        hipLaunchKernelGGL(k_tl_blockDiffers, dim3((unsigned)nP), dim3(kT), 0, nullptr, a, b, dBase, dLen, dT, dR, dDiff);
+        TL_OK(hipGetLastError());
+        differs.resize(nP);
+        TL_OK(hipMemcpy(differs.data(), dDiff, nP * 4, hipMemcpyDeviceToHost));
+        std::vector<std::vector<int32_t>> next;
+        size_t k = 0;
+        for (const auto& g : groups) {
+            std::vector<int32_t> rest;
+            for (size_t m = 1; m < g.size(); ++m, ++k) {
+                if (differs[k]) rest.push_back(g[m]);
+                else { out.rep[(size_t)g[m]] = g[0]; --out.distinct; }
+            }
+            if (rest.size() > 1) next.push_back(std::move(rest));
+        }
+        groups.swap(next);
+    }
     return 0;
 }
 
```

Measured after the change: 12.81 billion (median of 6 runs). +4.6%, better.
